# akloetgen/PARA-suite

Hardware: AMD Instinct MI355X
Metric: aligned reads/sec (10Mx50bp PAR-CLIP vs hg19-size genome) on MI355X; SAM bit-exact vs own CPU restatement (parity unpinned) (higher is better)
Workload: dtype u64

## Files before the change

para-suite_amd/csrc/ps_capi.hip:

```cpp
#include <hip/hip_runtime.h>
#include <chrono>
#include <condition_variable>
#include <deque>
#include <functional>
#include <map>
#include <mutex>
#include <thread>
#include <cstdio>
#include <cstdlib>
#include <cstring>
#include <string>
#include <fcntl.h>
#include <unistd.h>
#include "../../include/parasuite_hip.h"
#include "ps_pipeline.h"
#include "ps_bam.h"
#include "ps_host.h"

using namespace ps;

static thread_local std::string g_err;
static int fail(const std::string &m) { g_err = m; std::fprintf(stderr, "[parasuite-hip] error: %s\n", m.c_str()); return 1; }
#define PS_TRY try {
#define PS_CATCH_INT } catch (const std::exception &e) { return fail(e.what()); } catch (...) { return fail("unknown error"); }
// ... 201 lines not shown
int ps_ctx_blob(ps_ctx *x, int which, void **p, uint64_t *bytes)
{
    PS_TRY
        Index &ix = x->c.ix;
        if (which == 0) { *p = ix.blocks.p; *bytes = ix.blocks.n * sizeof(OccBlock); }
        else if (which == 1) { *p = ix.sa.p; *bytes = ix.sa.n * sizeof(uint32_t); }
        else if (which == 2) { *p = ix.pac.p; *bytes = ix.pac.n; }
        else throw Error("blob index out of range");
        return 0;
    PS_CATCH_INT
}
int64_t ps_ctx_meta(ps_ctx *x, char *buf, int64_t cap)
{
    try {
        std::string m = index_meta_serialize(x->c.ix);
        if (buf && cap >= (int64_t)m.size()) std::memcpy(buf, m.data(), m.size());
        return (int64_t)m.size();
    } catch (const std::exception &e) { fail(e.what()); return -1; }
}
ps_ctx *ps_ctx_from_blobs(const char *meta, int64_t meta_len, int device, void *const ptrs[3])
{
    ps_ctx *x = nullptr;
    PS_TRY
        x = new_ctx(device);
        Index &ix = x->c.ix;
        index_meta_deserialize(std::string(meta, (size_t)meta_len), ix);
        const bwtint primary = ix.view.primary; bwtint L2[5]; std::memcpy(L2, ix.view.L2, sizeof L2);
        const size_t nb = ix.view.n_blocks, ns = ix.view.n_sa, np = (size_t)ix.ref.l_pac / 4 + 1;
        ix.blocks.adopt((OccBlock *)ptrs[0], nb); ix.sa.adopt((uint32_t *)ptrs[1], Index::sa_words(ns)); ix.pac.adopt((uint8_t *)ptrs[2], np);
        ix.ref.pac.resize(np);
        PS_HIP(hipMemcpy(ix.ref.pac.data(), ix.pac.p, np, hipMemcpyDeviceToHost));
        ix.refresh_view();
        ix.view.primary = primary; std::memcpy(ix.view.L2, L2, sizeof L2);
        index_build_jump(ix, nullptr);
        return x;
    } catch (const std::exception &e) { delete x; fail(e.what()); return nullptr; } catch (...) { delete x; fail("unknown error"); return nullptr; }
}
int ps_ctx_fetch(ps_ctx *x, int which, void *dst, uint64_t bytes)
{
    PS_TRY
        void *p; uint64_t n;
        if (ps_ctx_blob(x, which, &p, &n)) return 1;
        if (bytes > n) throw Error("fetch larger than blob");
        PS_HIP(hipMemcpy(dst, p, bytes, hipMemcpyDeviceToHost));
        return 0;
    PS_CATCH_INT
}

int ps_ctx_export_blob(ps_ctx *x, int which, void *dst, uint64_t bytes)
{
    PS_TRY
        void *p; uint64_t n;
        if (ps_ctx_blob(x, which, &p, &n)) return 1;
        if (bytes != n) throw Error("export size differs from blob size");
        PS_HIP(hipMemcpy(dst, p, bytes, hipMemcpyDeviceToDevice));
        return 0;
    PS_CATCH_INT
}

ps_batch *ps_batch_from_fastq(ps_ctx *x, const char *fastq)
{
    PS_TRY
        require_device(x->c.device);
        ReadSet rs; load_reads(fastq, rs, x->c.host_threads);
        ps_batch *b = new ps_batch();
        b->b = batch_create(&x->c, std::move(rs));
        return b;
    PS_CATCH_PTR
}
ps_batch *ps_batch_from_codes(ps_ctx *x, int64_t n, int len, const uint8_t *codes)
{
    PS_TRY
        require_device(x->c.device);
        ReadSet rs; reads_from_codes(n, len, codes, rs);
        ps_batch *b = new ps_batch();
        b->b = batch_create(&x->c, std::move(rs));
        return b;
    PS_CATCH_PTR
}
void ps_batch_free(ps_batch *b) { delete b; }
int64_t ps_batch_n(ps_batch *b) { return b->b->rs.n; }
int ps_batch_search(ps_batch *b) { PS_TRY batch_search(*b->b); return 0; PS_CATCH_INT }
int ps_batch_select_hard(ps_batch *b, uint64_t before, uint64_t *after) { PS_TRY batch_select_hard(*b->b, before, after); return 0; PS_CATCH_INT }
int ps_batch_select_easy(ps_batch *b, int threads) { PS_TRY b->b->ctx->host_threads = threads > 0 ? threads : 1; batch_select_easy(*b->b, threads); return 0; PS_CATCH_INT }
int ps_batch_locate(ps_batch *b) { PS_TRY batch_locate(*b->b); return 0; PS_CATCH_INT }
int ps_batch_run(ps_batch *b, int threads)
{
    PS_TRY
        b->b->ctx->host_threads = threads > 0 ? threads : 1;
        batch_search(*b->b);
        batch_select_hard(*b->b, 0, nullptr);
        batch_select_easy(*b->b, threads);
        batch_locate(*b->b);
        return 0;
    PS_CATCH_INT
}
int ps_batch_write_sam(ps_batch *b, const char *path, int with_header, int threads)
{
    PS_TRY
        batch_write_sam(*b->b, path, with_header != 0, "@PG\tID:parasuite-hip\tPN:parasuite-hip\tVN:0.1", threads); return 0;
    PS_CATCH_INT
}
int ps_batch_n_aln(ps_batch *b, int32_t *out, int64_t cap)
{
    PS_TRY
        Batch &B = *b->b;
        for (int64_t g = 0; g < B.rs.n && g < cap; ++g) { int n; B.alns_of(g, n); out[g] = n; }
        return 0;
    PS_CATCH_INT
}
int64_t ps_batch_alns(ps_batch *b, int64_t read, ps_aln *out, int64_t cap)
{
    try {
        int n; const AlnRec *a = b->b->alns_of(read, n);
        for (int j = 0; j < n && j < cap; ++j) std::memcpy(&out[j], &a[j], sizeof(ps_aln));
        return n;
    } catch (const std::exception &e) { fail(e.what()); return -1; }
}
int ps_batch_hits(ps_batch *b, ps_hit *out, int64_t cap)
{
    PS_TRY
        Batch &B = *b->b;
        for (int64_t g = 0; g < B.rs.n && g < cap; ++g) {
            Hit h; B.hit_of(g, h); ps_hit &o = out[g];
            o.pos = h.type ? h.pos : -1; o.sa = h.sa; o.type = h.type; o.strand = h.strand; o.mapq = h.mapq; o.n_mm = h.n_mm; o.n_gapo = h.n_gapo;
            o.n_gape = h.n_gape; o.ref_shift = h.ref_shift; o.score = h.score; o.c1 = h.c1; o.c2 = h.c2; o.n_cigar = h.n_cigar; o.n_multi = h.n_multi;
            std::memset(o.cigar, 0, sizeof o.cigar); std::memcpy(o.cigar, h.cigar, sizeof h.cigar);
        }
        return 0;
    PS_CATCH_INT
}
int64_t ps_ctx_read_iters(ps_ctx *x, uint32_t *out, int64_t cap)
{
    const int64_t n = (int64_t)x->c.read_iters.size();
    for (int64_t i = 0; i < n && i < cap; ++i) out[i] = x->c.read_iters[i];
    return n;
}
int ps_batch_timing(ps_batch *b, ps_timing *o)
{
    PS_TRY
        const Timing &t = b->b->tm;
        o->ms_width = t.ms_width; o->ms_backtrack = t.ms_backtrack; o->ms_compact = t.ms_compact; o->ms_select = t.ms_select;
        o->ms_sa2pos = t.ms_sa2pos; o->ms_refine = t.ms_refine; o->ms_host_post = t.ms_host_post; o->ms_total = t.ms_total;
        o->ms_classify = t.ms_classify; o->ms_rows = t.ms_rows; o->ms_sel_hard = t.ms_sel_hard; o->ms_sel_easy = t.ms_sel_easy;
        o->n_width_launches = t.n_width_launches; o->n_backtrack_launches = t.n_backtrack_launches;
        o->n_overflow_tier1 = b->b->n_overflow[1]; o->n_overflow_tier2 = b->b->n_overflow[2];
        o->bt_begin_ms = t.bt_begin_ms; o->bt_end_ms = t.bt_end_ms;
        return 0;
    PS_CATCH_INT
}
int ps_batch_kstats(ps_batch *b, int which, ps_kstats *o)
{
    PS_TRY
        const KStats &k = which == 0 ? b->b->st_width : (which == 1 ? b->b->st_backtrack : b->b->st_sa2pos);
        o->occ_pairs = k.occ_pairs; o->occ_same_blk = k.occ_same_blk; o->nodes = k.nodes; o->pushes = k.pushes; o->pops = k.pops;
        o->lf_steps = k.lf_steps; o->iters = k.iters; o->exact_steps = k.exact_steps; return 0;
    PS_CATCH_INT
}

static const char *const PS_PG_LINE = "@PG\tID:parasuite-hip\tPN:parasuite-hip\tVN:0.1";
namespace {
struct ProfileSink { int min_mapq = 0, max_len = 0; std::string prefix; };
struct BamOut { int min_mapq = 0; bool sort = false, index = false; int level = 1; BamStats *stats = nullptr;
                bool by_name = false; BamFile *keep = nullptr; };
struct Resident { std::vector<ps_ctx *> xs; bool loaded = false; int n_index_loads = 0; };
struct PassIO { Resident *res = nullptr; std::vector<ReadSet> *reads = nullptr; std::function<void(Batch &)> after_piece; Resident *lanes_from = nullptr;
                int64_t n_reads = 0; double s_parse = 0, s_index = 0; };
}
static int map_core(int threads, const char *mm, const char *error_profile, const char *indel_profile,
                    const char *ref_fa, const char *fastq, const char *out_sam, const ProfileSink *sink, const BamOut *bam = nullptr, PassIO *io = nullptr)
{
    PS_TRY
        const bool verbose = std::getenv("PS_VERBOSE") != nullptr;
        const auto t_begin = std::chrono::steady_clock::now();
        auto since = [&]() { return std::chrono::duration<double>(std::chrono::steady_clock::now() - t_begin).count(); };
        const int nthr = threads > 0 ? threads : 1;
        std::vector<int> devs, dev_workers;
        int per_dev = 1;
        if (const char *e = std::getenv("PS_WORKERS_PER_GPU")) per_dev = std::max(1, std::min(std::atoi(e), (int)Ctx::N_WORK));
        {
            std::vector<int> named;
            if (const char *e = std::getenv("PARASUITE_GPU_IDS")) { for (const char *p = e; *p;) { named.push_back(std::atoi(p)); while (*p && *p != ',') ++p; if (*p == ',') ++p; } }
            else {
                int want = 1, have = 1;
                if (const char *e = std::getenv("PARASUITE_GPUS")) want = std::max(1, std::atoi(e));
                if (want > 1 && (hipGetDeviceCount(&have) != hipSuccess || have < 1)) return fail("no HIP device available");
                for (int g = 0; g < std::min(want, have); ++g) named.push_back(g);
            }
            if (named.empty()) named.push_back(0);
            for (int d : named) {
                size_t k = 0;
                while (k < devs.size() && devs[k] != d) ++k;
                if (k == devs.size()) { devs.push_back(d); dev_workers.push_back(0); }
                ++dev_workers[k];
            }
            for (int &w : dev_workers) w = std::min((int)Ctx::N_WORK, std::max(w, per_dev));
        }
        const int G = (int)devs.size();
        int n_workers = 0; for (int w : dev_workers) n_workers += w;
        size_t chunk_bytes = (size_t)1 << 30, first_bytes = 0, hungry_min = (size_t)128 << 20;
        if (const char *e = std::getenv("PS_CHUNK_MB")) { chunk_bytes = (size_t)std::max(1, std::atoi(e)) << 20; hungry_min = chunk_bytes; }
        else {
            FILE *f = io && io->reads ? nullptr : std::fopen(fastq, "rb");
            if (f) {
                if (fseeko(f, 0, SEEK_END) == 0) {
                    const off_t sz = ftello(f);
                    if (sz > 0) {
                        if (n_workers > 1) chunk_bytes = std::min(chunk_bytes, std::max<size_t>((size_t)16 << 20, ((size_t)sz + 2 * (size_t)n_workers - 1) / (2 * (size_t)n_workers) + ((size_t)64 << 10)));
                        hungry_min = std::min(chunk_bytes, std::max(hungry_min, (size_t)sz / 5));
                        if (bam) { chunk_bytes = std::min(chunk_bytes, std::max<size_t>((size_t)64 << 20, (size_t)sz / 4 + ((size_t)64 << 10))); hungry_min = std::min(hungry_min, chunk_bytes / 2); }
                    }
                }
                std::fclose(f);
            }
        }
        if (const char *e = std::getenv("PS_HUNGRY_MIN_MB")) hungry_min = (size_t)std::max(1, std::atoi(e)) << 20;
        if (const char *e = std::getenv("PS_FIRST_MB")) first_bytes = (size_t)std::max(1, std::atoi(e)) << 20;
        struct Piece { int64_t seq = 0; std::unique_ptr<Batch> b; };
        Chan<Piece> parsed;
        parsed.cap = (size_t)std::max(2, n_workers);
        Resident *const res = io ? io->res : nullptr;
        const bool preloaded = res && res->loaded;
        std::vector<ps_ctx *> xs((size_t)G, nullptr);
        if (res && !res->xs.empty()) { if (res->xs.size() != (size_t)G) return fail("internal: the resident contexts do not match the devices"); xs = res->xs; }
        auto close_all = [&]() { if (res) { res->xs = xs; return; } for (ps_ctx *c : xs) if (c) ps_ctx_close(c); };
        for (int g = 0; g < G; ++g) {
            if (!xs[g]) xs[g] = new_ctx(devs[g], false);
            if (error_profile && error_profile[0] ? ps_ctx_set_profile(xs[g], error_profile, indel_profile, mm)
                                                   : ps_ctx_set_stock(xs[g], mm && mm[0] ? mm : "0.04")) { const std::string m = g_err; close_all(); return fail(m); }
            xs[g]->c.host_threads = nthr;
            xs[g]->c.n_work = dev_workers[g];
        }
        if (res) res->xs = xs;
        if (io && io->lanes_from && io->lanes_from->xs.size() == (size_t)G)
            for (int g = 0; g < G; ++g) {
                Ctx &from = io->lanes_from->xs[g]->c, &to = xs[g]->c;
                if (from.device != to.device) continue;
                std::lock_guard<std::mutex> l1(from.work_mu), l2(to.work_mu);
                for (int w = 0; w < (int)Ctx::N_WORK; ++w) if (from.work[w] && !to.work[w]) to.work[w] = std::move(from.work[w]);
            }
        std::mutex mu; std::condition_variable cv;
        bool failed = false; std::string msg;
        int64_t next_select = 0, write_next = 0; uint64_t draws = 0;
        std::map<int64_t, std::unique_ptr<Batch>> done; int workers_left = n_workers;
        const size_t done_cap = (size_t)n_workers + 2;
        std::vector<int> index_state((size_t)G, preloaded ? 1 : 0);
        std::vector<int> attached((size_t)G, 0);
        auto fail_all = [&](const std::string &m) { { std::lock_guard<std::mutex> l(mu); if (!failed) { failed = true; msg = m; } } cv.notify_all(); parsed.abort(); };
        double t_parse = 0, t_write = 0, t_release = 0, t_index = 0, t_index_all = 0, t_profile = 0; std::vector<double> t_gpu((size_t)n_workers, 0.0);
        int64_t n_reads = 0, n_pieces = 0;
        Trash::trash().collect();
        std::thread parser([&]() {
            try {
                int64_t seq = 0;
                int pthr = nthr;
                if (const char *e = std::getenv("PS_PARSE_THREADS")) pthr = std::max(1, std::atoi(e));
                const std::function<bool()> hungry = [&]() { return parsed.hungry(); };
                if (io && io->reads) {
                    for (ReadSet &rs : *io->reads) { if (rs.n == 0) continue; Piece p; p.seq = seq++; p.b = batch_prepare(&xs[0]->c, std::move(rs), pthr); parsed.push(std::move(p)); }
                    io->reads->clear();
                } else
                load_reads_chunked(fastq, pthr, chunk_bytes, [&](ReadSet &&rs) {
                    Piece p; p.seq = seq++; p.b = batch_prepare(&xs[0]->c, std::move(rs), pthr);
                    parsed.push(std::move(p));
                }, first_bytes, &hungry, hungry_min);
                t_parse = since();
            } catch (const std::exception &e) { fail_all(e.what()); }
            parsed.close();
        });
        std::thread writer([&]() {
            try {
                bool first = true;
                SamScratch scratch;
                if (!bam) { const int fd = ::open(out_sam, O_WRONLY | O_CREAT | O_TRUNC, 0644); if (fd >= 0) ::close(fd); }
                std::unique_ptr<BamSink> bsink;
                std::unique_ptr<ProfileAccum> accum;
                for (;;) {
                    std::unique_ptr<Batch> b;
                    {
                        std::unique_lock<std::mutex> l(mu);
                        cv.wait(l, [&] { return failed || done.count(write_next) || (workers_left == 0 && done.empty()); });
                        if (failed) return;
                        auto it = done.find(write_next);
                        if (it == done.end()) break;
                        b = std::move(it->second); done.erase(it);
                    }
                    const auto t0 = std::chrono::steady_clock::now();
                    if (bam) {
                        if (!bsink) {
                            std::vector<std::pair<std::string, uint32_t>> refs;
                            for (const Contig &ct : b->ctx->ix.ref.contigs) refs.emplace_back(ct.name, (uint32_t)ct.len);
                            bsink.reset(new BamSink(sam_header(b->ctx->ix.ref, PS_PG_LINE), refs, out_sam, bam->sort, bam->index, nthr, bam->level, bam->by_name));
                        }
                        std::vector<std::string> enc; std::vector<std::vector<BamRec>> recs;
                        batch_bam_records(*b, bam->min_mapq, nthr, enc, recs);
                        bsink->add(enc, recs, (uint64_t)b->rs.n);
                    } else batch_write_sam(*b, out_sam, first, PS_PG_LINE, nthr, !first, &scratch);
                    t_write += std::chrono::duration<double>(std::chrono::steady_clock::now() - t0).count();
                    if (sink) {
                        const auto tp = std::chrono::steady_clock::now();
                        if (!accum) accum.reset(new ProfileAccum(xs[0]->c.device, xs[0]->c.ix, sink->max_len));
                        ProfRecords pr;
                        batch_profile_records(*b, sink->min_mapq, nthr, pr);
                        accum->add(pr);
                        t_profile += std::chrono::duration<double>(std::chrono::steady_clock::now() - tp).count();
                    }
                    if (io && io->after_piece) io->after_piece(*b);
// ... 457 lines not shown
```

para-suite_amd/csrc/ps_core.h:

```cpp
#pragma once
#include "ps_types.h"

namespace ps {

PS_HD uint32_t ps_popc(uint32_t x)
{
#ifdef __HIP_DEVICE_COMPILE__
    return (uint32_t)__popc(x);
#else
    return (uint32_t)__builtin_popcount(x);
#endif
}
PS_HD uint32_t pfx_mask32(int ns)
{
    return ns >= 32 ? 0xFFFFFFFFu : (ns <= 0 ? 0u : ((1u << ns) - 1u));
}

struct Blk { uint32_t x[16]; };

#ifdef __HIP_DEVICE_COMPILE__
#define PS_AS_GLOBAL(T, p) ((const __attribute__((address_space(1))) T *)(p))
#define PS_AS_GLOBAL_W(T, p) ((__attribute__((address_space(1))) T *)(p))
typedef uint32_t ps_u32x4 __attribute__((ext_vector_type(4)));
#endif

PS_HD int opaque_lane(int v)
{
#ifdef __HIP_DEVICE_COMPILE__
    asm volatile("" : "+v"(v));
#endif
    return v;
}

PS_HD void load_blk(const OccBlock *blocks, uint32_t b, Blk &o)
{
#ifdef __HIP_DEVICE_COMPILE__
    const __attribute__((address_space(1))) ps_u32x4 *p = PS_AS_GLOBAL(ps_u32x4, blocks + b);
    const ps_u32x4 a = p[0], c = p[1], d = p[2], e = p[3];
    o.x[0] = a.x; o.x[1] = a.y; o.x[2] = a.z; o.x[3] = a.w;
    o.x[4] = c.x; o.x[5] = c.y; o.x[6] = c.z; o.x[7] = c.w;
    o.x[8] = d.x; o.x[9] = d.y; o.x[10] = d.z; o.x[11] = d.w;
    o.x[12] = e.x; o.x[13] = e.y; o.x[14] = e.z; o.x[15] = e.w;
#else
    const uint32_t *p = reinterpret_cast<const uint32_t *>(blocks + b);
    for (int j = 0; j < 16; ++j) o.x[j] = p[j];
#endif
}
PS_HD void blk_count4(const Blk &b, int r, uint32_t cnt[4])
{
    uint32_t c1 = 0, c2 = 0, c3 = 0;
    const int q = r >> 5;
    const uint32_t part = (1u << (r & 31)) - 1u;
#pragma unroll
    for (int j = 0; j < 6; ++j) {
        const uint32_t m = j < q ? 0xFFFFFFFFu : (j == q ? part : 0u), lo = b.x[4 + j] & m, hi = b.x[10 + j] & m;
        c3 += ps_popc(lo & hi);
        c2 += ps_popc(hi & ~lo);
        c1 += ps_popc(lo & ~hi);
    }
    cnt[0] = b.x[0] + ((uint32_t)r - c1 - c2 - c3);
    cnt[1] = b.x[1] + c1; cnt[2] = b.x[2] + c2; cnt[3] = b.x[3] + c3;
}
PS_HD uint32_t blk_count1(const Blk &b, int r, int c)
{
    uint32_t n = 0;
    const uint32_t flo = (c & 1) ? 0u : 0xFFFFFFFFu, fhi = (c & 2) ? 0u : 0xFFFFFFFFu;
#pragma unroll
    for (int j = 0; j < 6; ++j) n += ps_popc((b.x[4 + j] ^ flo) & (b.x[10 + j] ^ fhi) & pfx_mask32(r - 32 * j));
    uint32_t base = c == 0 ? b.x[0] : (c == 1 ? b.x[1] : (c == 2 ? b.x[2] : b.x[3]));
    return base + n;
}
PS_HD int blk_sym(const Blk &b, int pos)
{
    uint32_t lo = 0, hi = 0; const int wi = pos >> 5;
#pragma unroll
    for (int j = 0; j < 6; ++j) { lo = (j == wi) ? b.x[4 + j] : lo; hi = (j == wi) ? b.x[10 + j] : hi; }
    return (int)(((lo >> (pos & 31)) & 1u) | (((hi >> (pos & 31)) & 1u) << 1));
}

PS_HD void blk_pack(OccBlock &b, const uint8_t *syms, int n, const uint32_t cnt[4])
{
    for (int c = 0; c < 4; ++c) b.cnt[c] = cnt[c];
    for (int j = 0; j < 6; ++j) {
        uint32_t lo = 0, hi = 0;
        for (int t = 0; t < 32; ++t) { int p = j * 32 + t; if (p < n) { lo |= (uint32_t)(syms[p] & 1) << t; hi |= (uint32_t)((syms[p] >> 1) & 1) << t; } }
        b.sym[j] = lo; b.sym[6 + j] = hi;
    }
}

PS_HD uint32_t sel4s(uint32_t v0, uint32_t v1, uint32_t v2, uint32_t v3, int c)
{
    const bool b0 = (c & 1) != 0, b1 = (c & 2) != 0;
    const uint32_t lo = b0 ? v1 : v0, hi = b0 ? v3 : v2;
    return b1 ? hi : lo;
}
PS_HD uint32_t sel4(const uint32_t v[4], int c) { return sel4s(v[0], v[1], v[2], v[3], c); }
PS_HD bwtint L2_of(const IndexView &ix, int c)
{
    const bool b0 = (c & 1) != 0, b1 = (c & 2) != 0;
    const bwtint lo = b0 ? ix.L2[1] : ix.L2[0], hi = b0 ? ix.L2[3] : ix.L2[2];
    return b1 ? hi : lo;
}
PS_HD uint32_t cost_word(const uint32_t pk[5], int s)
{
    const uint32_t w = sel4s(pk[0], pk[1], pk[2], pk[3], s);
    return s >= 4 ? pk[4] : w;
}
PS_HD int cost_of(const uint32_t pk[5], int s, int c) { return (int)((cost_word(pk, s) >> (8 * c)) & 0xffu); }

PS_HD bwtint row_to_stored(bwtint primary, bwtint row) { return row - (row >= primary ? 1u : 0u); }
PS_HD uint32_t blk_of(bwtint s, int &off)
{
    const uint32_t b = (uint32_t)(s >> 6) / 3u;
    off = (int)((uint32_t)s - b * (uint32_t)PS_BLK_SYMS);
    return b;
}
PS_HD uint32_t width32(bwtint k, bwtint l) { const bwtint w = l - k + 1; return w > 0xFFFFFFFFull ? 0xFFFFFFFFu : (uint32_t)w; }

struct LaneStats { uint32_t pairs, same, nodes, pushes, pops, iters, exact, lf; };

PS_HD void occ_pair4(const OccBlock *blocks, bwtint primary, bwtint k, bwtint l, uint32_t ck[4], uint32_t cl[4], LaneStats &st)
{
    int ol_ = 0, ok_ = 0;
    const uint32_t bl = blk_of(row_to_stored(primary, l), ol_);
    uint32_t bk = bl;
    bool need_k = k != 0;
    if (need_k) bk = blk_of(row_to_stored(primary, k - 1), ok_);
    Blk xl, xk;
    load_blk(blocks, bl, xl);
    bool other = need_k && bk != bl;
    if (other) load_blk(blocks, bk, xk);
    blk_count4(xl, ol_ + 1, cl);
#pragma unroll
    for (int j = 0; j < 16; ++j) xk.x[j] = other ? xk.x[j] : xl.x[j];
    blk_count4(xk, need_k ? ok_ + 1 : 0, ck);
    if (!need_k) { ck[0] = ck[1] = ck[2] = ck[3] = 0; }
    ++st.pairs;
    if (need_k && !other) ++st.same;
}
PS_HD void occ_pair1(const IndexView &ix, bwtint k, bwtint l, int c, uint32_t &ok, uint32_t &ol, LaneStats &st)
{
    int ol_ = 0, ok_ = 0;
    const uint32_t bl = blk_of(row_to_stored(ix.primary, l), ol_);
    uint32_t bk = bl;
    bool need_k = k != 0;
    if (need_k) bk = blk_of(row_to_stored(ix.primary, k - 1), ok_);
    Blk xl, xk;
    load_blk(ix.blocks, bl, xl);
    bool other = need_k && bk != bl;
    if (other) load_blk(ix.blocks, bk, xk);
    ol = blk_count1(xl, ol_ + 1, c);
    if (!need_k) ok = 0;
    else if (other) ok = blk_count1(xk, ok_ + 1, c);
    else ok = blk_count1(xl, ok_ + 1, c);
    ++st.pairs;
    if (need_k && !other) ++st.same;
}

PS_HD int read_base(const uint32_t *bases, const uint32_t *nmask, int n_reads, int r, int j)
{
    uint32_t w = bases[(size_t)(j >> 4) * n_reads + r];
    uint32_t m = nmask[(size_t)(j >> 5) * n_reads + r];
    return ((m >> (j & 31)) & 1u) ? 4 : (int)((w >> (2 * (j & 15))) & 3u);
}

PS_HD uint8_t cw_pack(int bid, bool eq) { return (uint8_t)((bid > 127 ? 127 : bid) | (eq ? 0x80 : 0)); }

struct WChain { bwtint k, l; int bid; uint32_t prev_w; };
PS_HD void wchain_init(const IndexView &ix, WChain &c) { c.k = 0; c.l = ix.seq_len; c.bid = 0; c.prev_w = 0xFFFFFFFFu; }
PS_HD void wchain_step(const IndexView &ix, WChain &c, int base, uint32_t &w_out, uint8_t &cw_out, bool first, LaneStats &st)
{
    if (base < 4) {
        uint32_t ok, ol;
        occ_pair1(ix, c.k, c.l, base, ok, ol, st);
        const bwtint l2 = L2_of(ix, base);
        c.k = l2 + ok + 1;
        c.l = l2 + ol;
    }
    if (c.k > c.l || base > 3) { c.k = 0; c.l = ix.seq_len; ++c.bid; }
    uint32_t w = width32(c.k, c.l);
    w_out = w;
    cw_out = cw_pack(c.bid, !first && w == c.prev_w);
    c.prev_w = w;
}

static const int PS_POP_TRIES = 1;
enum { M_FETCH = 0, M_POP = 1, M_EXACT = 2, M_EXPAND = 3, M_EXIT = 4, M_HIT = 5,
       M_GROW = 6 };

struct BtLane {
    int r, mode;
    bwtint k, l;
    int i, score, units, n_mm, n_gapo, n_gape, n_ins, n_del, state, ldp;
    bool have_cur;
    int best_score, max_units, n_aln, n_stack, status;
    unsigned long long best_cnt;
    unsigned long long bm0, bm1;
    uint32_t bump, free_head, iters0;
    uint32_t rn0, rn1;
    int len;
    uint32_t n_phantom;
    uint32_t cap;
    LaneStats st;
};

PS_HD int lm_ncw(int len) { return (len + 1 + 3) >> 2; }
PS_HD int lm_ncsw(int seed_len) { return seed_len > 0 ? (seed_len + 1 + 3) >> 2 : 0; }
PS_HD bool lm_nmask_in_regs(int len) { return len <= 64; }
PS_HD int lm_heads_off(int len, int seed_len) { return 4 * (lm_ncw(len) + lm_ncsw(seed_len) + ((len + 15) >> 4) + (lm_nmask_in_regs(len) ? 0 : ((len + 31) >> 5))); }
PS_HD int lm_bytes(int len, int seed_len, int n_buckets, bool wide)
{
    int n = lm_heads_off(len, seed_len) + (wide ? 0 : 2 * n_buckets);
    n = (n + 3) & ~3;
    if (((n >> 2) & 1) == 0) n += 4;
    return n;
}

static const int PS_JUMP_SLOT_WORDS = 8, PS_JUMP_MAX_LEVELS = 14;
PS_HD uint32_t jump_level_off(int d) { return 0x55555555u & ((1u << (2 * d)) - 1u); }
PS_HD size_t jump_words(int levels) { return (size_t)jump_level_off(levels) * PS_JUMP_SLOT_WORDS; }
PS_HD int jump_levels_for(bwtint seq_len) { int k = 0; while (k < PS_JUMP_MAX_LEVELS && (seq_len >> (2 * k)) >= 48) ++k; return k; }

struct BtHot {
    const OccBlock *blocks; bwtint primary;
    const uint32_t *jump; uint32_t jump_levels;
    uint32_t L2lo[4], L2hi;
    uint32_t s_pk[5], u_pk[5];
    uint32_t p0, p1, p2, p3;
    uint32_t inv_c_min, max_entries, pool_cap, n_reads, big_cap;
    uint32_t c_min;
    PS_HD int len() const { return (int)(p0 & 0xffu); }
    PS_HD int seed_len() const { return (int)((p0 >> 8) & 0xffu); }
    PS_HD int indel_end_skip() const { return (int)((p0 >> 16) & 0xffu); }
    PS_HD int max_del_occ() const { return (int)(p0 >> 24); }
    PS_HD int max_gapo() const { return (int)(p1 & 0xfu); }
    PS_HD int max_gape() const { return (int)((p1 >> 4) & 0xfu); }
    PS_HD bool mode_gape() const { return ((p1 >> 8) & 1u) != 0; }
    PS_HD bool use_seed() const { return ((p1 >> 9) & 1u) != 0; }
    PS_HD bool profile() const { return ((p1 >> 10) & 1u) != 0; }
    PS_HD bool has_big() const { return ((p1 >> 11) & 1u) != 0; }
    PS_HD int seed_units() const { return (int)((p1 >> 12) & 0xfffu); }
    PS_HD int u_tight() const { return (int)(p1 >> 24); }
    PS_HD int s_gapo_ins() const { return (int)(p2 & 0xffu); }
    PS_HD int s_gape() const { return (int)((p2 >> 8) & 0xffu); }
    PS_HD int s_gapo_del() const { return (int)((p2 >> 16) & 0xffu); }
    PS_HD int s_stop() const { return (int)(p2 >> 24); }
    PS_HD int u_gapo_ins() const { return (int)(p3 & 0xffu); }
    PS_HD int u_gape() const { return (int)((p3 >> 8) & 0xffu); }
    PS_HD int u_gapo_del() const { return (int)((p3 >> 16) & 0xffu); }
    PS_HD int n_buckets() const { return (int)(p3 >> 24); }
    PS_HD bwtint L2(int c) const
    { return (bwtint)L2lo[c] | ((bwtint)((L2hi >> c) & 1u) << 32); }
    PS_HD bwtint L2_dyn(int c) const
    { return (bwtint)sel4s(L2lo[0], L2lo[1], L2lo[2], L2lo[3], c) | ((bwtint)((L2hi >> c) & 1u) << 32); }
};
inline bool bt_hot_make(const BtArgs &a, BtHot &h)
{
    const Model &md = a.md;
    h.blocks = a.ix.blocks; h.primary = a.ix.primary; h.L2hi = 0;
    h.jump = a.ix.jump; h.jump_levels = a.ix.jump ? (uint32_t)a.ix.jump_levels : 0u;
    for (int c = 0; c < 4; ++c) { h.L2lo[c] = (uint32_t)a.ix.L2[c]; h.L2hi |= (uint32_t)((a.ix.L2[c] >> 32) & 1ull) << c; }
    h.L2hi |= (uint32_t)((a.ix.seq_len >> 32) & 1ull) << 4;
    for (int c = 0; c < 5; ++c) { h.s_pk[c] = md.s_mm_pk[c]; h.u_pk[c] = md.u_mm_pk[c]; }
    const int seed_units = md.max_seed_diff * md.u_tight;
    const bool ok = a.len >= 0 && a.len <= 255 && md.seed_len >= 0 && md.seed_len <= 255 && md.indel_end_skip >= 0 && md.indel_end_skip <= 255 &&
                    md.max_del_occ >= 0 && md.max_del_occ <= 255 && md.max_gapo >= 0 && md.max_gapo <= 15 && md.max_gape >= 0 && md.max_gape <= 15 &&
                    seed_units >= 0 && seed_units <= 4095 && md.u_tight >= 0 && md.u_tight <= 255 && md.s_stop >= 0 && md.s_stop <= 255 &&
                    md.s_gapo_ins >= 0 && md.s_gapo_ins <= 255 && md.s_gape >= 0 && md.s_gape <= 255 && md.s_gapo_del >= 0 && md.s_gapo_del <= 255 &&
                    md.u_gapo_ins >= 0 && md.u_gapo_ins <= 255 && md.u_gape >= 0 && md.u_gape <= 255 && md.u_gapo_del >= 0 && md.u_gapo_del <= 255 &&
                    md.n_buckets >= 0 && md.n_buckets <= 255 && md.max_entries >= 0 && md.inv_c_min >= 0 && md.max_units <= 255 && a.ix.L2[0] == 0;
    h.p0 = (uint32_t)a.len | ((uint32_t)md.seed_len << 8) | ((uint32_t)md.indel_end_skip << 16) | ((uint32_t)md.max_del_occ << 24);
    h.p1 = (uint32_t)md.max_gapo | ((uint32_t)md.max_gape << 4) | ((md.mode_gape ? 1u : 0u) << 8) | ((md.use_seed ? 1u : 0u) << 9) |
// ... 403 lines not shown
```

para-suite_amd/csrc/ps_kernels.h:

```cpp
#pragma once
#include <hip/hip_runtime.h>
#include "ps_types.h"
#include "ps_budget.h"

namespace ps {

static const int PS_MAX_CIGAR = 16;

struct WidthArgs {
    IndexView ix;
    int n_reads, len, seed_len, use_seed;
    const int32_t *lens;
    const uint32_t *bases; const uint32_t *nmask;
    uint32_t *w; uint32_t *cwb; uint32_t *cswb;
    KStats *stats;
};

struct EffortArgs {
    IndexView ix;
    int n_reads, len;
    const int32_t *lens;
    const uint32_t *bases; const uint32_t *nmask;
    uint32_t s_pk[5];
    int c_restart;
    uint32_t w_pin;
    uint8_t *est;
    uint16_t *est_ab;
};

struct EffortModelArgs {
    int n_reads, len;
    const int32_t *lens; const uint8_t *units_by_len;
    const uint32_t *bases; const uint32_t *nmask; const uint32_t *cwb;
    const uint8_t *est;
    uint32_t s_pk[5]; uint32_t inv_c_min;
    int max_units, u_tight, seed_units, use_seed, seed_len;
    int max_gapo, indel_end_skip, u_gapo_ins, u_gapo_del;
    int depth;
    float rows;
    int log_scale;
    uint8_t *key; float *pred;
};

struct RefineItem { int32_t read; bwtint rb; int32_t ref_shift; int32_t strand; };
struct RefineArgs {
    IndexView ix;
    int n_items, len, n_reads;
    const int32_t *lens;
    const uint32_t *bases; const uint32_t *nmask;
    const RefineItem *items;
    uint32_t *cigar; int32_t *n_cigar;
    uint8_t *zbuf; size_t z_per_block;
    int32_t *hebuf; size_t he_per_block;
};
inline size_t refine_he_words(int len) { return (size_t)(len + 2) * 64 * 2; }

static const size_t PS_LDS_PER_CU = 160 * 1024;
void set_dynamic_lds(const void *kernel, const char *name, size_t bytes);

void launch_width(const WidthArgs &a, hipStream_t s);
void launch_effort(const EffortArgs &a, hipStream_t s);
void launch_effort_model(const EffortModelArgs &a, hipStream_t s);
void launch_jump_build(const IndexView &ix, uint32_t *table, int levels, hipStream_t s);
bool launch_backtrack(const BtArgs &a, const BtArgs *d_args , BtArgs *h_stage ,
                      int n_blocks, int lm_stride, hipStream_t s, bool stats);
void launch_index_check(const IndexView &ix, unsigned long long *out , hipStream_t s);
void launch_sa2pos(const IndexView &ix, const bwtint *rows, bwtint *out, int n, KStats *stats, hipStream_t s);
void launch_refine(const RefineArgs &a, int n_blocks, hipStream_t s);
size_t order_sort_tmp_words(int n);
void launch_order_sort(const uint8_t *key, int n, uint32_t *tmp, int32_t *order, hipStream_t s);
void launch_class_ranks(const uint8_t *cls, long long n, const uint32_t *grp, uint32_t *e_before, uint32_t *h_before, hipStream_t s);

}
```

para-suite_amd/csrc/ps_kernels.hip:

```cpp
#include <hip/hip_runtime.h>
#include <algorithm>
#include <cstdlib>
#include <stdexcept>
#include <string>
#include "ps_core.h"
#include "ps_narrow.h"
#include "ps_kernels.h"

namespace ps {

static const int PS_Q_CHUNK = 64;
#ifndef PS_BT_WAVES
#define PS_BT_WAVES 4
#endif

__device__ __forceinline__ unsigned long long wave_sum(unsigned long long v)
{
    for (int o = 32; o > 0; o >>= 1) v += __shfl_xor(v, o, 64);
    return v;
}
__device__ __forceinline__ void flush_stats(KStats *ks, const LaneStats &st)
{
    if (!ks) return;
    unsigned long long v[8] = {st.pairs, st.same, st.nodes, st.pushes, st.pops, st.lf, st.iters, st.exact};
// ... 95 lines not shown
    const unsigned long long t_start = wall_clock64();
    int q_next = 0, q_end = 0;
    bool exhausted = false;
    for (;;) {
        const bool want = L.mode == M_FETCH;
        const unsigned long long wmask = __ballot(want), lmask = __ballot(L.mode != M_EXIT), hmask = __ballot(L.mode == M_HIT);
        if (lmask == 0) break;
        const bool stalled = (wmask | hmask) == lmask;
        const bool serve_hit = hmask != 0 && (__popcll(hmask) >= (int)hit_min || stalled);
        int fetch_r = -1;
        if (wmask) {
            const int cnt = __popcll(wmask);
            if (cnt >= (int)fetch_min || stalled) {
                const int rank = __popcll(wmask & lane_lt);
                int served = 0;
                while (served < cnt) {
                    if (q_next == q_end) {
                        if (exhausted) break;
                        unsigned int base = 0;
                        if (lane == 0) base = atomicAdd(queue, (unsigned int)PS_Q_CHUNK);
                        base = (unsigned int)__shfl((int)base, 0, 64);
                        if (base >= n_reads) { exhausted = true; break; }
                        q_next = (int)base;
                        q_end = (int)base + PS_Q_CHUNK < (int)n_reads ? (int)base + PS_Q_CHUNK : (int)n_reads;
                    }
                    const int take = q_end - q_next < cnt - served ? q_end - q_next : cnt - served;
                    if (want && rank >= served && rank < served + take) fetch_r = q_next + (rank - served);
                    q_next += take; served += take;
                }
                if (want && fetch_r < 0 && exhausted) fetch_r = (int)n_reads;
            }
        }
        bt_iter(a, h, L, m, fetch_r, serve_hit);
    }
    if (lane == 0) L.st.lf = (uint32_t)((wall_clock64() - t_start) >> 4);
    flush_stats(a.stats, L.st);
}


template <bool STATS, bool NB32>
__global__ void __launch_bounds__(256, PS_BT_WAVES) k_backtrack_n(const BtArgs *__restrict__ ap, BtHot hk, int lm_stride)
{
    const BtArgs &a = *ap;
    BtHot h; pin_hot(h, hk);
    uint32_t *const queue = reinterpret_cast<uint32_t *>(pin64(reinterpret_cast<unsigned long long>(a.queue)));
    const uint32_t n_reads = h.n_reads, fetch_min = pin32((uint32_t)a.fetch_min), hit_min = pin32((uint32_t)a.hit_min);
    extern __shared__ __attribute__((aligned(16))) uint8_t smem[];
    const int lane_g = blockIdx.x * blockDim.x + threadIdx.x;
    BtMem m;
    bt_mem_bind(m, smem + (size_t)threadIdx.x * lm_stride, h.len(), h.seed_len());
    uint8_t *const pool_private = reinterpret_cast<uint8_t *>(a.pool) + (size_t)lane_g * h.pool_cap * sizeof(Entry16);
    m.pool = pool_private;
    m.heads = nullptr;
    NLane L;
    nl_init(L);
    LaneStats st;
    ls_init(st);
    NtClock clk;
    for (int j = 0; j < 4; ++j) clk.tm[j] = 0;
    clk.t_last = 0;
#ifdef PS_STAMPS
    clk.t_last = __builtin_amdgcn_s_memtime();
#endif
    const int lane = threadIdx.x & 63;
    const unsigned long long t_start = STATS ? wall_clock64() : 0ull;
    uint32_t iters0 = 0;
    int q_next = 0, q_end = 0;
    bool exhausted = false;
    for (;;) {
        const int mode = nl_mode(L.ctl);
        const bool want = mode == M_FETCH;
        if (want && (L.ctl & NL_BIG)) {
            const unsigned int slot = (unsigned int)((reinterpret_cast<uint8_t *>(m.pool) - a.big_pool) / ((size_t)h.big_cap * sizeof(Entry16)));
            __threadfence();
            atomicExch(a.big_busy + slot, 0u);
            m.pool = pool_private;
            L.ctl &= ~NL_BIG;
        }
        const unsigned long long wmask = __ballot(want), lmask = __ballot(mode != M_EXIT), hmask = __ballot(mode == M_HIT);
        if (lmask == 0) break;
        const bool stalled = (wmask | hmask) == lmask;
        const bool serve_hit = hmask != 0 && (__popcll(hmask) >= (int)hit_min || stalled);
        int fetch_r = -1;
        if (wmask) {
            const int cnt = __popcll(wmask);
            if (cnt >= (int)fetch_min || stalled) {
                const int rank = (int)__builtin_amdgcn_mbcnt_hi((unsigned int)(wmask >> 32), __builtin_amdgcn_mbcnt_lo((unsigned int)wmask, 0u));
                int served = 0;
                while (served < cnt) {
                    if (q_next == q_end) {
                        if (exhausted) break;
                        unsigned int base = 0;
                        if (lane == 0) base = atomicAdd(queue, (unsigned int)PS_Q_CHUNK);
                        base = (unsigned int)__shfl((int)base, 0, 64);
                        if (base >= n_reads) { exhausted = true; break; }
                        q_next = (int)base;
                        q_end = (int)base + PS_Q_CHUNK < (int)n_reads ? (int)base + PS_Q_CHUNK : (int)n_reads;
                    }
                    const int take = q_end - q_next < cnt - served ? q_end - q_next : cnt - served;
                    if (want && rank >= served && rank < served + take) fetch_r = q_next + (rank - served);
                    q_next += take; served += take;
                }
                if (want && fetch_r < 0 && exhausted) fetch_r = (int)n_reads;
            }
        }
        unsigned long long gmask = __ballot(mode == M_GROW);
        while (gmask) {
            const int src = __ffsll((unsigned long long)gmask) - 1;
            gmask &= gmask - 1;
            const unsigned int n_big = a.n_big;
            unsigned int slot = n_big;
            if (lane == src) {
                unsigned int at = atomicAdd(a.big_next, 1u) % n_big;
                for (int tries = 0; tries < 256; ++tries) {
                    if (atomicCAS(a.big_busy + at, 0u, 1u) == 0u) { slot = at; break; }
                    at = at + 1u == n_big ? 0u : at + 1u;
                }
            }
            slot = (unsigned int)__shfl((int)slot, src, 64);
            const unsigned int n_copy = (unsigned int)__shfl((int)nl_bump(L), src, 64);
            const unsigned long long from = (unsigned long long)__shfl((long long)reinterpret_cast<unsigned long long>(m.pool), src, 64);
            if (slot < n_big) {
                const uint4 *sp = reinterpret_cast<const uint4 *>(from);
                uint4 *dp = reinterpret_cast<uint4 *>(a.big_pool + (size_t)slot * h.big_cap * sizeof(Entry16));
                for (unsigned int e = (unsigned int)lane; e < n_copy; e += 64u) dp[e] = sp[e];
                __threadfence();
                if (lane == src) { m.pool = dp; L.ctl = nl_set_mode(L.ctl | NL_BIG, M_EXPAND); }
            } else if (lane == src) L.ctl = nl_set_mode(nl_set_status(L.ctl, RS_OVERFLOW_POOL), M_POP);
        }
        nt_iter<STATS, NB32>(a, h, L, st, m, fetch_r, serve_hit, &clk);
        if (STATS && a.read_iters) {
            const int now = nl_mode(L.ctl);
            if (mode == M_FETCH && now != M_FETCH && now != M_EXIT) {
                iters0 = st.iters - 1u;
                const int len = nl_len(L), sl = h.seed_len();
                a.read_iters[PS_RI_WORDS * (size_t)L.r + 2] = (uint32_t)(m.cw[len - 1] & 0x7f) | ((h.use_seed() && sl > 0 && sl < len ? (uint32_t)(m.csw[sl - 1] & 0x7f) : 0u) << 8) | (a.est_ab ? (uint32_t)a.est_ab[L.r] << 16 : 0u);
                const uint32_t *cw32 = reinterpret_cast<const uint32_t *>(m.cw);
                for (int p = 0; p < 16; ++p) a.read_iters[PS_RI_WORDS * (size_t)L.r + 4 + p] = p < lm_ncw(len) ? cw32[p] : 0u;
            }
            if (mode != M_FETCH && mode != M_EXIT && now == M_FETCH) {
                uint32_t *ri = a.read_iters + PS_RI_WORDS * (size_t)L.r;
                ri[0] = st.iters - iters0; ri[1] = nl_bump(L);
                ri[3] = (uint32_t)nl_best_score(L) | ((uint32_t)nl_max_units(L) << 8) | ((uint32_t)nl_n_aln(L.ctl) << 16);
            }
        }
    }
    if (STATS) {
        if (lane == 0) st.lf = (uint32_t)((wall_clock64() - t_start) >> 4);
#ifdef PS_STAMPS
        st.nodes = lane == 0 ? (uint32_t)(clk.tm[0] >> 6) : 0; st.pushes = lane == 0 ? (uint32_t)(clk.tm[1] >> 6) : 0;
        st.pops = lane == 0 ? (uint32_t)(clk.tm[2] >> 6) : 0; st.exact = lane == 0 ? (uint32_t)(clk.tm[3] >> 6) : 0;
#endif
        flush_stats(a.stats, st);
    } else {
        st.nodes = st.pushes = st.pops = st.iters = st.exact = st.lf = 0;
        flush_stats(a.stats, st);
    }
}

__global__ void __launch_bounds__(256) k_sa2pos(IndexView ix, const bwtint *rows, bwtint *out, int n, KStats *stats)
{
    const int stride = gridDim.x * blockDim.x;
    int item = blockIdx.x * blockDim.x + threadIdx.x;
    LaneStats st = {0, 0, 0, 0, 0, 0, 0, 0};
    bool have = false; bwtint row = 0; uint32_t steps = 0;
    while (true) {
        if (!have) {
            if (item >= n) break;
            row = rows[item]; steps = 0; have = true;
        }
        if (!sa_walk_step(ix, row, steps, st)) {
            out[item] = (bwtint)steps + sa_sample(ix, row / (bwtint)ix.sa_intv);
            item += stride; have = false;
        }
    }
    flush_stats(stats, st);
}

__device__ __forceinline__ int text_sym(const IndexView &ix, bwtint p) { return p < ix.l_pac ? pac_base(ix.pac, p) : 3 - pac_base(ix.pac, 2 * ix.l_pac - 1 - p); }
__global__ void __launch_bounds__(256) k_index_check(IndexView ix, unsigned long long *out)
{
    unsigned long long rows = 0, bad_sym = 0, bad_sa = 0, longest = 0;
    const bwtint n_sa = ix.n_sa;
    for (bwtint t = (bwtint)blockIdx.x * blockDim.x + threadIdx.x; t < n_sa; t += (bwtint)gridDim.x * blockDim.x) {
        bwtint row = t * (bwtint)ix.sa_intv;
        bwtint p = t == 0 ? ix.seq_len : sa_sample(ix, t);
        unsigned long long steps = 0;
        do {
            if (p == 0) {
                if (row != ix.primary) ++bad_sym;
                row = 0; p = ix.seq_len;
            } else {
                if (row == ix.primary) { ++bad_sym; break; }
                int pos = 0;
                const uint32_t b = blk_of(row_to_stored(ix.primary, row), pos);
                Blk x;
                load_blk(ix.blocks, b, x);
                const int c = blk_sym(x, pos);
                if (c != text_sym(ix, p - 1)) ++bad_sym;
                row = L2_of(ix, c) + blk_count1(x, pos + 1, c);
                --p;
            }
            ++steps;
        } while ((row & (bwtint)(ix.sa_intv - 1)) != 0 && steps < 100000ull);
        if ((row & (bwtint)(ix.sa_intv - 1)) != 0) ++bad_sa;
        else {
            const bwtint t2 = row / (bwtint)ix.sa_intv;
            const bwtint want = t2 == 0 ? ix.seq_len : sa_sample(ix, t2);
            if (want != p) ++bad_sa;
        }
        rows += steps;
        if (steps > longest) longest = steps;
    }
    rows = wave_sum(rows); bad_sym = wave_sum(bad_sym); bad_sa = wave_sum(bad_sa);
    for (int o = 32; o > 0; o >>= 1) { const unsigned long long v = __shfl_xor(longest, o, 64); longest = v > longest ? v : longest; }
    if ((threadIdx.x & 63) == 0) { atomicAdd(out + 0, rows); atomicAdd(out + 1, bad_sym); atomicAdd(out + 2, bad_sa); atomicMax(out + 3, longest); }
}
void launch_index_check(const IndexView &ix, unsigned long long *out, hipStream_t s)
{
    hipLaunchKernelGGL(k_index_check, dim3(256 * 16), dim3(256), 0, s, ix, out);
}

__global__ void __launch_bounds__(64) k_refine(RefineArgs a)
{
    int32_t *H = a.hebuf + (size_t)blockIdx.x * a.he_per_block + threadIdx.x;
    int32_t *E = H + (size_t)(a.len + 2) * 64;
    uint8_t *z = a.zbuf + (size_t)blockIdx.x * a.z_per_block + threadIdx.x;
    for (int it = blockIdx.x * 64 + threadIdx.x; it < a.n_items; it += gridDim.x * 64) {
        RefineItem q = a.items[it];
        const int qlen = a.lens ? a.lens[q.read] : a.len;
        int tlen = qlen + q.ref_shift;
        int d = tlen - qlen; if (d < 0) d = -d;
        int w = (int)(d * 1.5); if (w < 50) w = 50;
        const int r = q.read, len = qlen, n_reads = a.n_reads;
        const uint32_t *bases = a.bases, *nmask = a.nmask;
        const int strand = q.strand;
        uint32_t cig[PS_MAX_CIGAR];
        int n = banded_global(len,
            [&](int j) { int b = read_base(bases, nmask, n_reads, r, strand ? len - 1 - j : j); return b > 3 ? 4 : (strand ? 3 - b : b); },
            tlen, a.ix.pac, q.rb, w, H, E, 64, z, 64, cig, PS_MAX_CIGAR);
        a.n_cigar[it] = n;
        for (int j = 0; j < PS_MAX_CIGAR; ++j) a.cigar[(size_t)it * PS_MAX_CIGAR + j] = j < n ? cig[j] : 0;
    }
}

void launch_width(const WidthArgs &a, hipStream_t s)
{
    int blocks = (a.n_reads + 255) / 256;
    if (blocks > 256 * 8) blocks = 256 * 8;
    if (blocks < 1) blocks = 1;
    hipLaunchKernelGGL(k_width, dim3(a.use_seed ? 2 * blocks : blocks), dim3(256), 0, s, a);
}
__global__ void __launch_bounds__(256) k_jump_level(BtHot h, uint32_t *table, bwtint seq_len, int d)
{
    const uint32_t n = 1u << (2 * d);
    for (uint32_t s = blockIdx.x * blockDim.x + threadIdx.x; s < n; s += gridDim.x * blockDim.x) jump_fill_slot(h, table, seq_len, d, s);
}
void launch_jump_build(const IndexView &ix, uint32_t *table, int levels, hipStream_t s)
{
    BtArgs a{};
    a.ix = ix; a.ix.jump = nullptr; a.ix.jump_levels = 0;
    BtHot h;
    (void)bt_hot_make(a, h);
    for (int d = 0; d < levels; ++d) {
        const uint32_t n = 1u << (2 * d);
        const int blocks = (int)std::min<uint32_t>((n + 255u) / 256u, 256u * 16u);
        hipLaunchKernelGGL(k_jump_level, dim3(blocks), dim3(256), 0, s, h, table, ix.seq_len, d);
    }
}
bool launch_backtrack(const BtArgs &a_in, const BtArgs *d_args, BtArgs *h_stage, int n_blocks, int lm_stride, hipStream_t s, bool stats)
{
    BtArgs &a = *h_stage;
    a = a_in;
    const char *ej = std::getenv("PS_JUMP");
    const bool stats_plain = stats && !std::getenv("PS_STATS_JUMP");
    if (stats_plain || a.wide || (ej && std::atoi(ej) == 0)) { a.ix.jump = nullptr; a.ix.jump_levels = 0; }
    BtHot h;
    if (!bt_hot_make(a, h)) return false;
    (void)hipMemcpyAsync(const_cast<BtArgs *>(d_args), &a, sizeof(BtArgs), hipMemcpyHostToDevice, s);
    const size_t lds = (size_t)256 * lm_stride;
    const bool nb32 = a.md.n_buckets <= 32;
    typedef void (*KernelN)(const BtArgs *, BtHot, int);
    const KernelN kn = stats ? (nb32 ? k_backtrack_n<true, true> : k_backtrack_n<true, false>) : (nb32 ? k_backtrack_n<false, true> : k_backtrack_n<false, false>);
    const void *fn = a.wide ? reinterpret_cast<const void *>(k_backtrack_wide) : reinterpret_cast<const void *>(kn);
    set_dynamic_lds(fn, a.wide ? "k_backtrack_wide" : "k_backtrack_n", lds);
    if (a.wide) hipLaunchKernelGGL(k_backtrack_wide, dim3(n_blocks), dim3(256), lds, s, d_args, h, lm_stride);
    else hipLaunchKernelGGL(kn, dim3(n_blocks), dim3(256), lds, s, d_args, h, lm_stride);
    return true;
}
void launch_sa2pos(const IndexView &ix, const bwtint *rows, bwtint *out, int n, KStats *stats, hipStream_t s)
{
    int blocks = (n + 255) / 256;
    if (blocks > 256 * 8) blocks = 256 * 8;
    if (blocks < 1) blocks = 1;
    hipLaunchKernelGGL(k_sa2pos, dim3(blocks), dim3(256), 0, s, ix, rows, out, n, stats);
}
void launch_refine(const RefineArgs &a, int n_blocks, hipStream_t s)
{
    if (!a.hebuf || a.he_per_block < refine_he_words(a.len)) throw std::runtime_error("k_refine: H/E scratch missing or too small");
    hipLaunchKernelGGL(k_refine, dim3(n_blocks), dim3(64), 0, s, a);
}
void set_dynamic_lds(const void *kernel, const char *name, size_t bytes)
{
    if (bytes <= 48 * 1024) return;
    const std::string what = std::string(name) + ": " + std::to_string(bytes) + " B of dynamic LDS";
    if (bytes > PS_LDS_PER_CU) throw std::runtime_error(what + " requested, a CU has " + std::to_string(PS_LDS_PER_CU));
// ... 6 lines not shown
```

para-suite_amd/csrc/ps_narrow.h:

```cpp
#pragma once
#include "ps_core.h"

namespace ps {

PS_HD int nw_i(uint32_t wa) { return (int)(wa & 0xffu); }
PS_HD int nw_ldp(uint32_t wa) { return (int)((wa >> 8) & 0xffu); }
PS_HD int nw_mm(uint32_t wa) { return (int)((wa >> 16) & 0xffu); }
PS_HD int nw_state(uint32_t wa) { return (int)((wa >> 24) & 3u); }
PS_HD int nw_gapo(uint32_t wa) { return (int)((wa >> 26) & 7u); }
PS_HD int nw_gape(uint32_t wa) { return (int)(wa >> 29); }
PS_HD int nw_ins(uint32_t wb) { return (int)(wb & 7u); }
PS_HD int nw_del(uint32_t wb) { return (int)((wb >> 3) & 7u); }
PS_HD uint32_t nw_c(uint32_t wb) { return (wb >> 6) & 7u; }
PS_HD int nw_score(uint32_t wb) { return (int)((wb >> 9) & 0x7fu); }
static const uint32_t NW_KEEP = 0xFCFF0000u;
static const uint32_t NW_C_MASK = 7u << 6;
static const uint32_t NW_ROOT_C = 4u;

PS_HD int nl_mode(uint32_t ctl) { return (int)(ctl & 7u); }
PS_HD uint32_t nl_set_mode(uint32_t ctl, int mode) { return (ctl & ~7u) | (uint32_t)mode; }
static const uint32_t NL_HAVE_CUR = 8u, NL_STATUS = 7u << 4, NL_BIG = 1u << 7;
PS_HD int nl_status(uint32_t ctl) { return (int)((ctl >> 4) & 7u); }
PS_HD uint32_t nl_set_status(uint32_t ctl, int s) { return (ctl & ~NL_STATUS) | ((uint32_t)s << 4); }
PS_HD int nl_n_aln(uint32_t ctl) { return (int)(ctl >> 16); }

struct NLane {
    uint32_t kr, lr, wa, wb;
    uint32_t ctl;
    int r;
    uint32_t lim;
    uint32_t nsb;
    uint32_t n_phantom;
    uint32_t fh;
    uint32_t bm0, bm1;
    uint32_t rn0, rn1;
};
PS_HD int nl_best_score(const NLane &L) { return (int)(L.lim & 0xffu); }
PS_HD int nl_max_units(const NLane &L) { return (int)((L.lim >> 8) & 0xffu); }
PS_HD int nl_len(const NLane &L) { return (int)((L.lim >> 16) & 0xffu); }
PS_HD int nl_n_stack(const NLane &L) { return (int)(L.nsb & 0xffffu); }
PS_HD uint32_t nl_bump(const NLane &L) { return L.nsb >> 16; }
PS_HD uint32_t nl_phantom(const NLane &L) { return L.n_phantom & 0x00FFFFFFu; }
PS_HD int nl_est(const NLane &L) { return (int)(L.n_phantom >> 24); }

PS_HD void nl_init(NLane &L)
{
    L.kr = L.lr = L.wa = L.wb = 0; L.ctl = (uint32_t)M_FETCH; L.r = 0; L.lim = 0; L.nsb = 0;
    L.n_phantom = 0; L.fh = 0xffffu; L.bm0 = L.bm1 = 0; L.rn0 = L.rn1 = 0;
}
PS_HD void ls_init(LaneStats &st) { st.pairs = st.same = st.nodes = st.pushes = st.pops = st.iters = st.exact = st.lf = 0; }
PS_HD uint32_t ps_mul24(uint32_t x, uint32_t y)
{
#ifdef __HIP_DEVICE_COMPILE__
    return __umul24(x, y);
#else
    return x * y;
#endif
}

struct NtClock { unsigned long long tm[4]; unsigned long long t_last; };
#if defined(PS_STAMPS) && defined(__HIP_DEVICE_COMPILE__)
#define PS_USTAMP(clk, slot) do { if (STATS && (clk)) { const unsigned long long t_ = __builtin_amdgcn_s_memtime(); (clk)->tm[slot] += t_ - (clk)->t_last; (clk)->t_last = t_; } } while (0)
#else
#define PS_USTAMP(clk, slot) do { } while (0)
#endif

PS_HD bwtint nt_base(const BtHot &h, uint32_t c)
{
    return (bwtint)sel4s(h.L2lo[0], h.L2lo[1], h.L2lo[2], h.L2lo[3], (int)c) | ((bwtint)((h.L2hi >> c) & 1u) << 32);
}
PS_HD int nt_units(const BtHot &h, uint32_t wa, uint32_t wb)
{
    return h.profile() ? nw_score(wb) : nw_mm(wa) + nw_gapo(wa) + (h.mode_gape() ? nw_gape(wa) : 0);
}

PS_HD void blk_count4b(const Blk &b, int r, uint32_t cnt[4])
{
    uint32_t A = 0, B = 0, C = 0;
    const int q = r >> 5;
    const uint32_t part = (1u << (r & 31)) - 1u;
#pragma unroll
    for (int j = 0; j < 6; ++j) {
        const uint32_t m = j < q ? 0xFFFFFFFFu : (j == q ? part : 0u), lo = b.x[4 + j] & m, hi = b.x[10 + j] & m;
        A += ps_popc(lo); B += ps_popc(hi); C += ps_popc(lo & hi);
    }
    cnt[0] = b.x[0] + ((uint32_t)r - A - B + C);
    cnt[1] = b.x[1] + (A - C); cnt[2] = b.x[2] + (B - C); cnt[3] = b.x[3] + C;
}

#ifndef PS_OCC_COND
#define PS_OCC_COND 1
#endif
template <bool STATS>
PS_HD void nt_occ(const BtHot &h, uint32_t c, uint32_t kr, uint32_t lr, uint32_t ck[4], uint32_t cl[4], LaneStats &st)
{
    const bwtint base = nt_base(h, c);
    const bool need_k = c != NW_ROOT_C;
    int ol_ = 0, ok_ = 0;
    const uint32_t bl = blk_of(row_to_stored(h.primary, base + lr), ol_);
    uint32_t bk = blk_of(row_to_stored(h.primary, base + (bwtint)(need_k ? kr - 1u : 0u)), ok_);
    bk = need_k ? bk : 0u;
    const int rk = need_k ? ok_ + 1 : 0;
    Blk xl, xk;
    load_blk(h.blocks, bl, xl);
    if (PS_OCC_COND) {
        const bool other = bk != bl;
        if (other) load_blk(h.blocks, bk, xk);
        blk_count4b(xl, ol_ + 1, cl);
#pragma unroll
        for (int j = 0; j < 16; ++j) xk.x[j] = other ? xk.x[j] : xl.x[j];
    } else { load_blk(h.blocks, bk, xk); blk_count4b(xl, ol_ + 1, cl); }
    blk_count4b(xk, rk, ck);
    ++st.pairs; if (need_k && bk == bl) ++st.same;
    (void)STATS;
}

PS_HD int nt_depth(int len, uint32_t wa, uint32_t wb) { return len - nw_i(wa) - (int)(wb & 7u) + (int)((wb >> 3) & 7u); }
PS_HD void nt_jump(const BtHot &h, int d, uint32_t sidx, uint32_t ck[4], uint32_t cl[4])
{
    const uint32_t *sl = h.jump + (size_t)(jump_level_off(d) + sidx) * PS_JUMP_SLOT_WORDS;
#ifdef __HIP_DEVICE_COMPILE__
    const ps_u32x4 a = *PS_AS_GLOBAL(ps_u32x4, sl), b = *PS_AS_GLOBAL(ps_u32x4, sl + 4);
    ck[0] = a.x; cl[0] = a.y; ck[1] = a.z; cl[1] = a.w; ck[2] = b.x; cl[2] = b.y; ck[3] = b.z; cl[3] = b.w;
#else
    for (int c = 0; c < 4; ++c) { ck[c] = sl[2 * c]; cl[c] = sl[2 * c + 1]; }
#endif
}
PS_HD void jump_fill_slot(const BtHot &h, uint32_t *table, bwtint seq_len, int d, uint32_t s)
{
    uint32_t c = NW_ROOT_C, kr = 0, lr = (uint32_t)seq_len;
    bool empty = false;
    if (d > 0) {
        const uint32_t *ps = table + (size_t)(jump_level_off(d - 1) + (s >> 2)) * PS_JUMP_SLOT_WORDS;
        c = s & 3u;
        empty = ps[2 * c] >= ps[2 * c + 1];
        kr = ps[2 * c] + 1u; lr = ps[2 * c + 1];
    }
    uint32_t ck[4] = {0, 0, 0, 0}, cl[4] = {0, 0, 0, 0};
    LaneStats st;
    if (!empty) nt_occ<false>(h, c, kr, lr, ck, cl, st);
    uint32_t *out = table + (size_t)(jump_level_off(d) + s) * PS_JUMP_SLOT_WORDS;
    for (int j = 0; j < 4; ++j) { out[2 * j] = ck[j]; out[2 * j + 1] = cl[j]; }
}

PS_HD int nt_seq_at(const BtMem &m, const NLane &L, int j, int len, int max_len)
{
    const int p = len - 1 - j;
    const uint32_t b = (m.rb[p >> 4] >> (2 * (p & 15))) & 3u;
    const uint32_t nw = lm_nmask_in_regs(max_len) ? (p < 32 ? L.rn0 : L.rn1) : m.rn[p >> 5];
    return ((nw >> (p & 31)) & 1u) ? 4 : 3 - (int)b;
}

PS_HD void nt_heads_init(BtMem &m, int n_buckets)
{
    uint32_t *hw = reinterpret_cast<uint32_t *>(m.heads16);
    for (int p = 0; p < (n_buckets + 1) >> 1; ++p) hw[p] = 0xFFFFFFFFu;
}
PS_COLD void nt_restart_without_estimate(const BtArgs &a, NLane &L, BtMem &m)
{
    L.ctl = (L.ctl & NL_BIG) | (uint32_t)M_POP | NL_HAVE_CUR;
    L.kr = 0; L.lr = (uint32_t)a.ix.seq_len; L.wa = (uint32_t)nl_len(L); L.wb = NW_ROOT_C << 6;
    L.lim = (L.lim & 0x00FFFF00u) | 0xffu;
    L.nsb = 0; L.bm0 = L.bm1 = 0; L.fh = 0xffffu; L.n_phantom = 0xFF000000u;
    nt_heads_init(m, a.md.n_buckets);
}
PS_HD void nt_finish_read(const BtArgs &a, NLane &L)
{
    a.n_aln[L.r] = nl_n_aln(L.ctl);
    a.status[L.r] = (uint8_t)nl_status(L.ctl);
    L.ctl = nl_set_mode(L.ctl, M_FETCH);
}

PS_COLD void nt_hit(const BtArgs &a, NLane &L, BtMem &m)
{
    const Model &md = a.md;
    const uint32_t c = nw_c(L.wb);
    if (a.ix.jump && c != NW_ROOT_C) {
        const int d = nt_depth(nl_len(L), L.wa, L.wb);
        if (d < a.ix.jump_levels) {
            const uint32_t *ps = a.ix.jump + (size_t)(jump_level_off(d - 1) + (L.kr >> 2)) * PS_JUMP_SLOT_WORDS;
            L.kr = ps[2 * c] + 1u; L.lr = ps[2 * c + 1];
        }
    }
    const bwtint base = c == NW_ROOT_C ? (a.ix.seq_len & ~(bwtint)0xFFFFFFFFull) : a.ix.L2[c];
    const bwtint k = base + L.kr, l = base + L.lr;
    const int score = nw_score(L.wb), n_gapo = nw_gapo(L.wa);
    const int units = md.profile ? score : nw_mm(L.wa) + n_gapo + (md.mode_gape ? nw_gape(L.wa) : 0);
    const int n_aln = nl_n_aln(L.ctl);
    if (n_aln == 0) {
        if (units > nl_est(L)) { nt_restart_without_estimate(a, L, m); return; }
        int t = units + md.u_tight;
        const int own = nl_max_units(L);
        t = t > own ? own : t;
        L.lim = (L.lim & 0x00FF0000u) | (uint32_t)score | ((uint32_t)t << 8);
    }
    if (score == nl_best_score(L)) {
        const unsigned long long s = (unsigned long long)(L.lim >> 24) + (unsigned long long)(l - k) + 1ull;
        L.lim = (L.lim & 0x00FFFFFFu) | ((s > 255ull ? 255u : (uint32_t)s) << 24);
    } else if ((int)(L.lim >> 24) > md.max_top2) { nt_finish_read(a, L); return; }
    AlnRec *out = a.alns + (size_t)L.r * a.aln_cap;
    if (n_gapo) {
        for (int j = 0; j < n_aln; ++j)
            if (out[j].k == k && out[j].l == l) return;
    }
    {
        const uint32_t shadow = a.ix.seq_len > 0xFFFFFFFFull ? 0xFFFFFFFFu : (uint32_t)a.ix.seq_len;
        uint32_t x = (uint32_t)(l - k + 1), j = 0, prev = 0;
        const int lim = nw_ldp(L.wa);
        for (int i = 0; i < lim; ++i) {
            size_t off = (size_t)i * a.n_reads + L.r;
            uint32_t w = a.w[off];
            int bid = m.cw[i] & 0x7f;
            if (w > x) { w -= x; a.w[off] = w; }
            else if (w == x) {
                if (bid > 1 && nl_phantom(L)) L.ctl = nl_set_status(L.ctl, RS_OVERFLOW_POOL);
                bid = 1; w = shadow - (++j); a.w[off] = w;
            }
            m.cw[i] = cw_pack(bid, i > 0 && w == prev);
            prev = w;
        }
        if (lim > 0) {
            uint32_t w = a.w[(size_t)lim * a.n_reads + L.r];
            m.cw[lim] = cw_pack(m.cw[lim] & 0x7f, w == prev);
        }
    }
    if (n_aln >= a.aln_cap) { L.ctl = nl_set_status(L.ctl, RS_OVERFLOW_ALN); nt_finish_read(a, L); return; }
    AlnRec rec;
    rec.k = k; rec.l = l; rec.score = (uint16_t)score; rec.units = (uint16_t)units;
    rec.n_mm = (uint8_t)nw_mm(L.wa); rec.n_gapo = (uint8_t)n_gapo; rec.n_gape = (uint8_t)nw_gape(L.wa);
    rec.n_ins = (uint8_t)nw_ins(L.wb); rec.n_del = (uint8_t)nw_del(L.wb);
    for (int j = 0; j < 7; ++j) rec.pad[j] = 0;
    out[n_aln] = rec;
    L.ctl += 1u << 16;
}

PS_COLD bool nt_fetch(const BtArgs &a, NLane &L, BtMem &m, int q)
{
    const Model &md = a.md;
    const int r = a.order ? a.order[q] : q;
    const int len = a.lens ? a.lens[r] : a.len;
    L.r = r;
    L.ctl = (uint32_t)M_FETCH;
    L.n_phantom = 0xFF000000u;
    const int max_units = (a.lens && a.units_by_len) ? (int)a.units_by_len[len] : md.max_units;
    L.lim = 0xffu | ((uint32_t)max_units << 8) | ((uint32_t)len << 16);
    {
        const int ncw = lm_ncw(len), ncsw = lm_ncsw(md.seed_len);
        uint32_t *cw32 = reinterpret_cast<uint32_t *>(m.cw), *csw32 = reinterpret_cast<uint32_t *>(m.csw);
        for (int p = 0; p < ncw; ++p) cw32[p] = a.cwb[(size_t)p * a.n_reads + r];
        for (int p = 0; p < ncsw; ++p) csw32[p] = a.cswb[(size_t)p * a.n_reads + r];
        const int nbw = (len + 15) >> 4;
        for (int p = 0; p < nbw; ++p) m.rb[p] = a.bases[(size_t)p * a.n_reads + r];
    }
    int nNu = 0;
    L.rn0 = L.rn1 = 0;
    const int nmw = (len + 31) >> 5;
    for (int p = 0; p < nmw; ++p) {
        uint32_t w = a.nmask[(size_t)p * a.n_reads + r];
        if (lm_nmask_in_regs(a.len)) { if (p == 0) L.rn0 = w; else L.rn1 = w; }
        else m.rn[p] = w;
        nNu += (int)ps_popc(w) * (int)(md.u_mm_pk[4] & 0xffu);
    }
    if (nNu > max_units) { nt_finish_read(a, L); return false; }
    L.kr = 0; L.lr = (uint32_t)a.ix.seq_len; L.wa = (uint32_t)len; L.wb = NW_ROOT_C << 6;
    L.ctl |= NL_HAVE_CUR;
    L.nsb = 0; L.bm0 = L.bm1 = 0; L.fh = 0xffffu;
    {
        int e = 255;
        if (a.cap_est) { e = (int)a.est[r] - (a.cap_est - 1); if (e < 0) e = 0; }
        L.n_phantom = (uint32_t)(e + md.u_tight < max_units ? e : 255) << 24;
    }
    nt_heads_init(m, md.n_buckets);
    return true;
}

PS_HD uint32_t nt_slot(NLane &L)
{
    const uint32_t fr = L.fh;
    const bool reuse = fr != 0xffffu;
    const uint32_t idx = reuse ? fr : (L.nsb >> 16);
    L.nsb += reuse ? 1u : 0x10001u;
    L.fh = 0xffffu;
    return idx;
}
PS_HD void nt_push(NLane &L, BtMem &m, uint32_t kr, uint32_t lr, uint32_t wa, uint32_t wb)
{
    const int score = nw_score(wb);
    const uint32_t idx = nt_slot(L);
    const uint32_t next = (uint32_t)m.heads16[score];
    Entry16 e; e.k = kr; e.l = lr; e.a = wa; e.b = wb | (next << 16);
    store16(reinterpret_cast<Entry16 *>(m.pool) + idx, e);
    m.heads16[score] = (uint16_t)idx;
    if (score < 32) L.bm0 |= 1u << score; else L.bm1 |= 1u << (score - 32);
}

template <bool NB32>
PS_HD void nt_pop(NLane &L, BtMem &m)
{
#ifdef __HIP_DEVICE_COMPILE__
    const int b = (NB32 || L.bm0) ? __ffs((int)L.bm0) - 1 : 32 + __ffs((int)L.bm1) - 1;
#else
    const int b = (NB32 || L.bm0) ? __builtin_ctz(L.bm0) : 32 + __builtin_ctz(L.bm1);
#endif
    const uint32_t hd = m.heads16[b];
    Entry16 e;
    load16(reinterpret_cast<const Entry16 *>(m.pool) + hd, e);
    const uint32_t next = e.b >> 16;
    L.fh = hd;
    m.heads16[b] = (uint16_t)next;
    if (next == PS_NIL16) { if (NB32 || b < 32) L.bm0 &= ~(1u << b); else L.bm1 &= ~(1u << (b - 32)); }
    L.kr = e.k; L.lr = e.l; L.wa = e.a; L.wb = e.b & 0xffffu;
    L.nsb -= 1u;
}

template <bool STATS, bool NB32>
PS_HD int nt_head(const BtArgs &a, const BtHot &h, NLane &L, LaneStats &st, BtMem &m, int fetch_r, bool serve_hit)
{
    int mode = nl_mode(L.ctl);
    if (mode == M_EXIT || mode == M_GROW) return 0;
    if (STATS) ++st.iters;
    if (mode == M_HIT) {
        if (!serve_hit) return 0;
        L.ctl = nl_set_mode(L.ctl, M_POP);
        { NLane t = L; nt_hit(a, t, m); L = t; }
        return 0;
    }
    if (mode == M_FETCH) {
        if (fetch_r < 0) return 0;
        if (fetch_r >= (int)h.n_reads) { L.ctl = nl_set_mode(L.ctl, M_EXIT); return 0; }
        { NLane t = L; const bool ok = nt_fetch(a, t, m, fetch_r); L = t; if (!ok) return 0; }
        L.ctl = nl_set_mode(L.ctl, M_POP);
        mode = M_POP;
    }
    if (mode == M_POP) {
        const int n_virtual = nl_n_stack(L) + ((L.ctl & NL_HAVE_CUR) ? 1 : 0);
        if (nl_phantom(L) && (long long)n_virtual + (long long)nl_phantom(L) > (long long)h.max_entries) {
            L.ctl = nl_set_status(L.ctl, RS_OVERFLOW_POOL); nt_finish_read(a, L); return 0;
        }
        if (n_virtual == 0 && nl_est(L) != 255 && nl_n_aln(L.ctl) == 0 && nl_status(L.ctl) == RS_OK) { NLane t = L; nt_restart_without_estimate(a, t, m); L = t; return 0; }
        if (n_virtual == 0 || n_virtual > (int)h.max_entries || nl_status(L.ctl) != RS_OK) { nt_finish_read(a, L); return 0; }
        if (L.ctl & NL_HAVE_CUR) L.ctl &= ~NL_HAVE_CUR;
        else { nt_pop<NB32>(L, m); if (STATS) ++st.pops; }
        L.ctl = nl_set_mode(L.ctl, M_POP);
        const int score = nw_score(L.wb), i1 = nw_i(L.wa);
        if (score > nl_best_score(L) + h.s_stop()) { nt_finish_read(a, L); return 0; }
        const int rem = nl_max_units(L) - nt_units(h, L.wa, L.wb);
        if (rem < 0) return 0;
        const int mleft = (int)(ps_mul24((uint32_t)rem, h.inv_c_min) >> 16);
        if (i1 > 0 && mleft < (int)(m.cw[i1 - 1] & 0x7f)) return 0;
        if (i1 == 0) { L.ctl = nl_set_mode(L.ctl, M_HIT); return 0; }
        const int st_ = nw_state(L.wa);
        mode = (mleft == 0 && (st_ == ST_M || h.mode_gape() || nw_gape(L.wa) == h.max_gape())) ? M_EXACT : M_EXPAND;
    }
    return mode;
}

struct NtStep { uint32_t ck[4], cl[4]; uint32_t cw_i, cw_im1, cs_i, cs_im1; int s, i; bool in_seed, tm, ctm; };

template <bool STATS>
PS_HD void nt_step_occ(const BtHot &h, NLane &L, LaneStats &st, BtMem &m, NtStep &q)
{
    const int len = nl_len(L), max_len = h.len();
    const int i = nw_i(L.wa) - 1;
    q.i = i;
    q.cw_i = m.cw[i]; q.cw_im1 = m.cw[i > 0 ? i - 1 : 0];
    const int ii = i - (len - h.seed_len());
    q.in_seed = h.use_seed() && len > h.seed_len() && ii > 0;
    q.cs_i = q.in_seed ? m.csw[ii] : 0u; q.cs_im1 = q.in_seed ? m.csw[ii - 1] : 0u;
    q.s = nt_seq_at(m, L, i, len, max_len);
    const int depth = nt_depth(len, L.wa, L.wb);
    q.tm = depth < (int)h.jump_levels; q.ctm = depth + 1 < (int)h.jump_levels;
    if (!q.tm) nt_occ<STATS>(h, nw_c(L.wb), L.kr, L.lr, q.ck, q.cl, st);
    else nt_jump(h, depth, L.kr, q.ck, q.cl);
}

template <bool STATS, bool NB32>
PS_HD void nt_tail(const BtHot &h, NLane &L, LaneStats &st, BtMem &m, const NtStep &q, int mode)
{
    const int len = nl_len(L), i = q.i, s = q.s;
    const uint32_t cw_i = q.cw_i, cw_im1 = q.cw_im1, cs_i = q.cs_i, cs_im1 = q.cs_im1;
    const bool in_seed = q.in_seed, tm = q.tm, ctm = q.ctm;
    uint32_t ck[4], cl[4];
#pragma unroll
    for (int c = 0; c < 4; ++c) { ck[c] = q.ck[c]; cl[c] = q.cl[c]; }
    if (mode == M_EXACT) {
        if (STATS) ++st.exact;
        L.ctl = nl_set_mode(L.ctl, M_POP);
        if (s > 3) return;
        const uint32_t ok = sel4(ck, s), ol = sel4(cl, s);
        if (ok >= ol) return;
        L.kr = ctm ? (L.kr << 2) | (uint32_t)s : ok + 1u; L.lr = ctm ? ol - ok : ol; L.wa -= 1u; L.wb = (L.wb & ~NW_C_MASK) | ((uint32_t)s << 6);
        L.ctl = nl_set_mode(L.ctl, i == 0 ? M_HIT : M_EXACT);
        return;
    }
    if (STATS) ++st.nodes;
    const uint32_t cap = (L.ctl & NL_BIG) ? h.big_cap : h.pool_cap;
    if (nl_bump(L) + 9u > cap) {
        if (!(L.ctl & NL_BIG) && h.has_big()) { L.ctl = nl_set_mode(L.ctl, M_GROW); return; }
        L.ctl = nl_set_mode(nl_set_status(L.ctl, cap >= 65535u ? RS_OVERFLOW_DEEP : RS_OVERFLOW_POOL), M_POP); return;
    }
    const int max_units = nl_max_units(L);
    const int e_un = nt_units(h, L.wa, L.wb), e_sc = nw_score(L.wb);
    const int rem = max_units - e_un;
    const uint32_t inv = h.inv_c_min;
    const int mleft = (int)(ps_mul24((uint32_t)rem, inv) >> 16);
    const int srem = h.seed_units() - e_un;
    const int m_seed = srem <= 0 ? 0 : (int)(ps_mul24((uint32_t)srem, inv) >> 16);
    bool allow_diff = true, allow_M = true;
    const int bnd_same = i > 0 ? (int)(cw_im1 & 0x7f) : 0;
    const int bnd_del = (int)(cw_i & 0x7f);
    if (i > 0) {
        if (bnd_same > mleft - 1) allow_diff = false;
        else if (bnd_same == mleft - 1 && bnd_del == mleft - 1 && (cw_i & 0x80u)) allow_M = false;
        if (in_seed) {
            const int s1 = (int)(cs_im1 & 0x7f), s0 = (int)(cs_i & 0x7f);
            if (s1 > m_seed - 1) allow_diff = false;
            else if (s1 == m_seed - 1 && s0 == m_seed - 1 && (cs_i & 0x80u)) allow_M = false;
        }
    }
    const int e_go = nw_gapo(L.wa), e_ge = nw_gape(L.wa), e_st = nw_state(L.wa);
    const int tmp = e_go + e_ge;
    const bool gap_ok = allow_diff && i >= h.indel_end_skip() + tmp && len - i >= h.indel_end_skip() + tmp;
    const bool from_m = e_st == ST_M, from_i = e_st == ST_I, from_d = e_st == ST_D;
    const uint32_t wa_keep = L.wa & NW_KEEP, pos2 = (uint32_t)i | ((uint32_t)i << 8);
    const uint32_t wb0 = L.wb & 0x1ffu;
    const uint32_t pkr = L.kr, plr = L.lr;
    const int need_same = (int)ps_mul24((uint32_t)bnd_same, h.c_min), need_del = (int)ps_mul24((uint32_t)bnd_del, h.c_min);
    const int cap_rem = nl_est(L) - e_sc, ut = h.u_tight();
    const int cap_same = cap_rem + (ut > need_same ? ut - need_same : 0), cap_del = cap_rem + (ut > need_del ? ut - need_del : 0);
    const int thr_same = (rem - need_same) < cap_same ? (rem - need_same) : cap_same, thr_del = (rem - need_del) < cap_del ? (rem - need_del) : cap_del;
    uint32_t phantom = 0, gmask = 0;
    int sc[9];
    uint32_t wa_i, wa_d;
    {
        const bool open = from_m && e_go < h.max_gapo(), ext = from_i && e_ge < h.max_gape();
        const int c = open ? h.u_gapo_ins() : h.u_gape();
        sc[0] = e_sc + (open ? h.s_gapo_ins() : h.s_gape());
        const bool cand = gap_ok && (open || ext) && c <= rem, go = cand && c <= thr_same;
        gmask |= go ? 1u : 0u;
        phantom += (cand && !go) ? 1u : 0u;
        wa_i = wa_keep + pos2 + ((uint32_t)ST_I << 24) + (open ? 1u << 26 : 1u << 29);
    }
    {
        const uint32_t occ = tm ? plr : plr - pkr + 1u;
        const bool open = from_m && e_go < h.max_gapo();
        const bool ext = from_d && e_ge < h.max_gape() && ((e_ge + e_go) * h.u_tight() < max_units || occ < (uint32_t)h.max_del_occ());
        const int c = open ? h.u_gapo_del() : h.u_gape();
        const int scd = e_sc + (open ? h.s_gapo_del() : h.s_gape());
        const bool cand = gap_ok && (open || ext) && c <= rem, go = cand && c <= thr_del;
        const uint32_t ne = (ck[0] < cl[0] ? 2u : 0u) | (ck[1] < cl[1] ? 4u : 0u) | (ck[2] < cl[2] ? 8u : 0u) | (ck[3] < cl[3] ? 16u : 0u);
        gmask |= go ? ne : 0u;
        if (cand && !go) phantom += ps_popc(ne);
        sc[1] = sc[2] = sc[3] = sc[4] = scd;
        wa_d = wa_keep + ((uint32_t)(i + 1) | ((uint32_t)(i + 1) << 8)) + ((uint32_t)ST_D << 24) + (open ? 1u << 26 : 1u << 29);
    }
    const bool do_mm = allow_diff && allow_M;
    const uint32_t s_word = cost_word(h.s_pk, s), u_word = h.profile() ? s_word : cost_word(h.u_pk, s);
    uint32_t xk[4], xl[4];
#pragma unroll
    for (int j = 1; j <= 4; ++j) {
        const int c = (s + j) & 3;
        xk[j - 1] = sel4(ck, c); xl[j - 1] = sel4(cl, c);
        sc[4 + j] = 0;
        if (j < 4 || s > 3) {
            const int cu = (int)((u_word >> (8 * c)) & 0xffu);
            sc[4 + j] = e_sc + (int)((s_word >> (8 * c)) & 0xffu);
            const bool cand = do_mm && xk[j - 1] < xl[j - 1] && cu <= rem, go = cand && cu <= thr_same;
            gmask |= go ? 1u << (4 + j) : 0u;
            phantom += (cand && !go) ? 1u : 0u;
        }
    }
    const uint32_t n_push = ps_popc(gmask), fr = L.fh;
    const bool reuse = fr != 0xffffu && n_push != 0u;
    const uint32_t slot0 = (L.nsb >> 16) - (reuse ? 1u : 0u);
    L.nsb += n_push + ((n_push - (reuse ? 1u : 0u)) << 16);
    L.fh = n_push ? 0xffffu : fr;
    if (STATS) st.pushes += n_push;
    uint32_t idx[9], raw[9];
#pragma unroll
    for (int j = 0; j < 9; ++j) {
        idx[j] = 0; raw[j] = 0;
        if ((gmask >> j) & 1u) {
            const uint32_t rank = ps_popc(gmask & ((1u << j) - 1u));
            idx[j] = (reuse && rank == 0u) ? fr : slot0 + rank;
            raw[j] = m.heads16[sc[j]];
            m.heads16[sc[j]] = (uint16_t)idx[j];
            if (NB32 || sc[j] < 32) L.bm0 |= 1u << sc[j]; else L.bm1 |= 1u << (sc[j] - 32);
        }
    }
#ifdef __HIP_DEVICE_COMPILE__
    asm volatile("" : "+v"(raw[0]), "+v"(raw[1]), "+v"(raw[2]), "+v"(raw[3]), "+v"(raw[4]), "+v"(raw[5]), "+v"(raw[6]), "+v"(raw[7]), "+v"(raw[8]));
#endif
    Entry16 *const pool = reinterpret_cast<Entry16 *>(m.pool);
#define NT_NEXT(j) (raw[j] << 16)
    if (gmask & 1u) { Entry16 e; e.k = pkr; e.l = plr; e.a = wa_i; e.b = (wb0 + 1u) | ((uint32_t)sc[0] << 9) | NT_NEXT(0); store16(pool + idx[0], e); }
    {
        const uint32_t wb_d = ((wb0 & 0x3fu) + (1u << 3)) | ((uint32_t)sc[1] << 9);
#pragma unroll
        for (int c = 0; c < 4; ++c)
            if ((gmask >> (1 + c)) & 1u) { Entry16 e; e.k = ctm ? (pkr << 2) | (uint32_t)c : ck[c] + 1u; e.l = ctm ? cl[c] - ck[c] : cl[c]; e.a = wa_d; e.b = wb_d | ((uint32_t)c << 6) | NT_NEXT(1 + c); store16(pool + idx[1 + c], e); }
    }
    {
// ... 34 lines not shown
```

para-suite_amd/csrc/ps_pipeline.h:

```cpp
#pragma once
#include <functional>
#include <map>
#include <memory>
#include <mutex>
#include "ps_host.h"
#include "ps_reads.h"
#include "ps_bam.h"

namespace ps {

static const int PS_HIT_CIGAR = 8;
struct Multi { int64_t pos; bwtint row; int32_t gap, mm, ref_shift, strand, n_cigar; uint32_t cigar[PS_MAX_CIGAR]; };
struct Hit {
    int64_t pos; bwtint sa;
    int32_t type, strand, mapq, n_mm, n_gapo, n_gape, ref_shift, score, c1, c2, n_cigar;
    int32_t multi_begin, n_multi;
    uint32_t cigar[PS_HIT_CIGAR];
};

static const uint8_t PS_CLS_HOST = 4;
struct SelRec { bwtint sa; int32_t c1, c2; uint8_t type, n_mm, n_gapo, n_gape; int8_t ref_shift; uint8_t score, pad[2]; };
struct FinRec { int64_t pos; uint8_t strand, mapq, type, pad[5]; };
struct DevCigar { int64_t g; int32_t n; uint32_t c[PS_HIT_CIGAR]; };
struct SubRead { int64_t g = 0, easy_before = 0, hard_before = 0; uint8_t cls = 0; const AlnRec *alns = nullptr; int32_t n_alns = 0; Hit hit; };

struct Timing {
    double ms_width = 0, ms_backtrack = 0, ms_compact = 0, ms_select = 0, ms_sa2pos = 0, ms_refine = 0, ms_host_post = 0, ms_total = 0, ms_classify = 0, ms_rows = 0, ms_sel_hard = 0, ms_sel_easy = 0;
    int n_width_launches = 0, n_backtrack_launches = 0;
    double bt_begin_ms = 0, bt_end_ms = 0;
};

void *pin_cache_take(size_t need, size_t &got);
void pin_cache_give(void *p, size_t bytes);
void pin_cache_release();
struct PinBuf {
    void *p = nullptr; size_t bytes = 0;
    PinBuf() {}
    PinBuf(const PinBuf &) = delete;
    PinBuf &operator=(const PinBuf &) = delete;
    ~PinBuf() { if (p) pin_cache_give(p, bytes); }
    void *get(size_t need) { if (need > bytes) { if (p) pin_cache_give(p, bytes); p = nullptr; bytes = 0; p = pin_cache_take(need, bytes); } return p; }
};

struct Work {
    hipStream_t stream = nullptr;
    std::map<std::string, DevBuf<uint8_t>> ws; std::map<std::string, PinBuf> pin;
    template <class T> T *ws_get(const std::string &name, size_t count) {
        DevBuf<uint8_t> &b = ws[name];
        const size_t need = count * sizeof(T);
        if (b.n < need) b.alloc(need + need / 8);
        return reinterpret_cast<T *>(b.p);
    }
    template <class T> T *pin_get(const std::string &name, size_t count) { return reinterpret_cast<T *>(pin[name].get(count * sizeof(T) + 64)); }
    Work() {}
    Work(const Work &) = delete;
    Work &operator=(const Work &) = delete;
    ~Work() { if (stream) (void)hipStreamDestroy(stream); }
};

struct Ctx {
    int device = 0;
    hipStream_t stream = nullptr;
    hipEvent_t ref_event = nullptr;
    Index ix;
    Options opt;
    int bt_blocks = 0;
    uint32_t pool_cap[3] = {16384, 65535, 2000064};
    int aln_cap[3] = {8, 256, 65536};
    int aln_cap_short = 32;
    bool want_kstats = false;
    bool want_read_iters = false; std::vector<uint32_t> read_iters;
    int n_big = 4096;
    int fetch_min = 8, hit_min = 1;
    int host_threads = 8;
    static const int N_WORK = 4;
    std::unique_ptr<Work> work[N_WORK];
    int n_work = 1, next_work = 0;
    Work *take_work();
    Work *work_at(int i);
    std::mutex work_mu;
    ~Ctx();
};

struct Bin {
    int len = 0; Model md;
    bool ragged = false;
    std::vector<int32_t> lens; DevBuf<int32_t> d_lens;
    std::vector<int32_t> ids;
    DevBuf<uint32_t> bases, nmask, w; DevBuf<uint8_t> cwb, cswb, status; DevBuf<AlnRec> alns; DevBuf<int32_t> n_aln;
    RawVec<uint32_t> h_bases, h_nmask;
    DevBuf<int32_t> d_ids;
    DevBuf<AlnRec> d_alns; DevBuf<int32_t> d_n_aln; DevBuf<uint8_t> d_status; int aln_cap = 0;
    bool host_alns_valid = false;
    std::vector<int32_t> h_n_aln; std::vector<uint32_t> h_off; std::vector<AlnRec> h_alns;
    std::map<int32_t, std::vector<AlnRec>> overflow;
    int n_bw = 0, n_mw = 0;
};

struct Batch {
    Ctx *ctx = nullptr;
    Work *wk = nullptr;
    int work_index = -1;
    ReadSet rs;
    std::vector<Bin> bins;
    std::vector<int32_t> read_bin, read_local;
    DevBuf<uint8_t> d_class; DevBuf<uint32_t> d_eb, d_hb; DevBuf<bwtint> d_rows, d_pos; DevBuf<SelRec> d_sel; DevBuf<FinRec> d_fin;
    PinBuf p_class, p_sel, p_fin, p_grp;
    uint8_t *h_class = nullptr; SelRec *h_sel = nullptr; FinRec *h_fin = nullptr;
    uint32_t *h_grp = nullptr;
    std::vector<SubRead> sub; std::vector<Multi> multis; std::vector<DevCigar> dev_cigars;
    std::vector<std::unique_ptr<PinBuf>> sub_alns;
    int64_t n_class1 = 0, n_hard = 0;
    std::vector<uint64_t> hard_draws_cum;
    uint64_t draws_in = 0, draws_out = 0;
    DevBuf<KStats> d_stats; KStats st_width{}, st_backtrack{}, st_sa2pos{};
    Timing tm;
    int64_t n_overflow[3] = {0, 0, 0};
    bool searched = false, selected_hard = false, selected = false, located = false;
    const AlnRec *alns_of(int64_t g, int &n);
    void ensure_host_alns();
    void hit_of(int64_t g, Hit &h) const;
    void release_device();
};

std::unique_ptr<Batch> batch_create(Ctx *ctx, ReadSet &&rs);
std::unique_ptr<Batch> batch_prepare(Ctx *ctx, ReadSet &&rs, int threads);
void batch_upload(Batch &b);
void batch_search(Batch &b);
void batch_select_hard(Batch &b, uint64_t draws_before, uint64_t *draws_after);
void batch_select_easy(Batch &b, int threads);
void ctx_release_device(Ctx &c);
void reserve_search_workspace(Ctx *ctx, int work_index);
void batch_locate(Batch &b);
void batch_bam_records(const Batch &b, int min_mapq, int threads, std::vector<std::string> &enc, std::vector<std::vector<BamRec>> &recs);
std::string sam_header(const RefSeq &ref, const char *pg_line);
struct SamScratch { std::vector<std::string> bufs[2]; };
void batch_write_sam(Batch &b, const char *path, bool header, const char *pg_line, int threads, bool append = false, SamScratch *scratch = nullptr);
void batch_profile_records(const Batch &b, int min_mapq, int threads, ProfRecords &out);

}
```

para-suite_amd/csrc/ps_pipeline.hip:

```cpp
#include <hip/hip_runtime.h>
#include <mutex>
#include <optional>
#include <hipcub/hipcub.hpp>
#include <algorithm>
#include <atomic>
#include <chrono>
#include <cmath>
#include <cstdio>
#include <cstring>
#include <functional>
#include <thread>
#include "ps_pipeline.h"
#include "ps_par.h"
#include "ps_core.h"

namespace ps {

typedef std::chrono::steady_clock Clock;
static double ms_since(Clock::time_point t0) { return std::chrono::duration<double, std::milli>(Clock::now() - t0).count(); }

void require_device(int device)
{
    int n = 0;
    hipError_t e = hipGetDeviceCount(&n);
// ... 46 lines not shown
            return p;
        }
    }
    const size_t want = need + need / 8 + 4096;
    void *p = nullptr;
    PS_HIP(hipHostMalloc(&p, want, hipHostMallocDefault));
    got = want;
    return p;
}
void pin_cache_give(void *p, size_t bytes)
{
    if (!p) return;
    PinCache &c = pin_cache();
    {
        std::lock_guard<std::mutex> l(c.mu);
        if (c.held + bytes <= PinCache::CAP) { c.kept.emplace_back(p, bytes); c.held += bytes; return; }
    }
    (void)hipHostFree(p);
}
void pin_cache_release()
{
    PinCache &c = pin_cache();
    std::vector<std::pair<void *, size_t>> all;
    { std::lock_guard<std::mutex> l(c.mu); all.swap(c.kept); c.held = 0; }
    for (auto &e : all) (void)hipHostFree(e.first);
}

void Batch::release_device()
{
    for (Bin &bin : bins) {
        bin.bases.release(); bin.nmask.release(); bin.w.release(); bin.cwb.release(); bin.cswb.release(); bin.status.release();
        bin.alns.release(); bin.n_aln.release(); bin.d_lens.release(); bin.d_ids.release();
        bin.d_alns.release(); bin.d_n_aln.release(); bin.d_status.release();
    }
    d_class.release(); d_eb.release(); d_hb.release(); d_rows.release(); d_pos.release(); d_sel.release(); d_fin.release(); d_stats.release();
    searched = false;
}

std::unique_ptr<Batch> batch_prepare(Ctx *ctx, ReadSet &&rs_in, int threads)
{
    const auto t_prep0 = std::chrono::steady_clock::now();
    struct PrepTimes { double bins = 0, sort = 0, pack = 0; } pt;
    std::unique_ptr<Batch> b(new Batch());
    b->ctx = ctx; b->rs = std::move(rs_in);
    const ReadSet &rs = b->rs;
    std::vector<int> class_of_len;
    std::map<std::vector<int>, int> bin_of_class;
    b->read_bin.resize((size_t)rs.n); b->read_local.resize((size_t)rs.n);
    for (int64_t g = 0; g < rs.n; ++g) {
        const int len = rs.len[g];
        if (len < 1) throw Error("empty read in input");
        if ((size_t)len >= class_of_len.size()) class_of_len.resize((size_t)len + 64, -1);
        int cls = class_of_len[(size_t)len];
        if (cls < 0) {
            Model md; std::string err;
            if (!make_model(ctx->opt, len, md, err)) throw Error(err);
            const std::vector<int> key = {md.max_gapo};
            auto bc = bin_of_class.find(key);
            if (bc == bin_of_class.end()) { bc = bin_of_class.emplace(key, (int)b->bins.size()).first; b->bins.emplace_back(); }
            cls = class_of_len[(size_t)len] = bc->second;
        }
        Bin &bin = b->bins[(size_t)cls];
        if (bin.len && bin.len != len) bin.ragged = true;
        if (len > bin.len) bin.len = len;
        b->read_bin[g] = cls; b->read_local[g] = (int32_t)bin.ids.size();
        bin.ids.push_back((int32_t)g);
    }
    pt.bins = std::chrono::duration<double>(std::chrono::steady_clock::now() - t_prep0).count();
    for (Bin &bin : b->bins) {
        std::string err;
        if (!make_model(ctx->opt, bin.len, bin.md, err)) throw Error(err);
        if (!std::getenv("PS_KEEP_ORDER")) {
            const size_t n = bin.ids.size();
            const int nt = par_threads(n, threads);
            std::vector<uint32_t> key(n), key2(n); std::vector<int32_t> id2(n);
            par_for(n, nt, [&](size_t r0, size_t r1, int) {
                for (size_t r = r0; r < r1; ++r) {
                    const uint8_t *sq = rs.seq.data() + rs.off[bin.ids[r]];
                    const int kb = rs.len[bin.ids[r]] < 16 ? rs.len[bin.ids[r]] : 16;
                    uint32_t k = 0;
                    for (int j = 0; j < kb; ++j) k = (k << 2) | (uint32_t)(sq[j] & 3);
                    key[r] = k << (2 * (16 - kb));
                }
            });
            std::vector<size_t> cnt((size_t)nt * 256);
            for (int sh = 0; sh < 32; sh += 8) {
                std::fill(cnt.begin(), cnt.end(), 0);
                par_for(n, nt, [&](size_t r0, size_t r1, int t) { size_t *c = cnt.data() + (size_t)t * 256; for (size_t r = r0; r < r1; ++r) ++c[(key[r] >> sh) & 0xff]; });
                size_t at = 0;
                for (int d = 0; d < 256; ++d) for (int t = 0; t < nt; ++t) { const size_t c = cnt[(size_t)t * 256 + d]; cnt[(size_t)t * 256 + d] = at; at += c; }
                par_for(n, nt, [&](size_t r0, size_t r1, int t) {
                    size_t *c = cnt.data() + (size_t)t * 256;
                    for (size_t r = r0; r < r1; ++r) { const size_t p = c[(key[r] >> sh) & 0xff]++; key2[p] = key[r]; id2[p] = bin.ids[r]; }
                });
                key.swap(key2); bin.ids.swap(id2);
            }
            par_for(n, nt, [&](size_t r0, size_t r1, int) { for (size_t r = r0; r < r1; ++r) b->read_local[bin.ids[r]] = (int32_t)r; });
        }
        const size_t n = bin.ids.size();
        pt.sort = std::chrono::duration<double>(std::chrono::steady_clock::now() - t_prep0).count() - pt.bins - pt.pack;
        bin.n_bw = (bin.len + 15) / 16; bin.n_mw = (bin.len + 31) / 32;
        bin.h_bases.resize((size_t)bin.n_bw * n); bin.h_nmask.resize((size_t)bin.n_mw * n);
        bin.lens.resize(n);
        {
            const int nt = std::max(1, std::min(threads, 64));
            auto pack = [&](int t) {
                const size_t r_end = n * (t + 1) / nt, AHEAD = 12;
                for (size_t r = n * t / nt; r < r_end; ++r) {
                    if (r + 2 * AHEAD < r_end) { const int32_t g2 = bin.ids[r + 2 * AHEAD]; __builtin_prefetch(&rs.off[g2]); __builtin_prefetch(&rs.len[g2]); }
                    if (r + AHEAD < r_end) { const uint8_t *q = rs.seq.data() + rs.off[bin.ids[r + AHEAD]]; __builtin_prefetch(q); __builtin_prefetch(q + 63); }
                    const uint8_t *s = rs.seq.data() + rs.off[bin.ids[r]];
                    const int rl = rs.len[bin.ids[r]];
                    bin.lens[r] = rl;
                    for (int p = 0; p < bin.n_bw; ++p) {
                        uint32_t wd = 0;
                        const int j1 = std::min(rl, 16 * p + 16);
                        for (int j = 16 * p; j < j1; ++j) if (s[j] <= 3) wd |= (uint32_t)s[j] << (2 * (j & 15));
                        bin.h_bases[(size_t)p * n + r] = wd;
                    }
                    for (int p = 0; p < bin.n_mw; ++p) {
                        uint32_t wd = 0;
                        const int j1 = std::min(rl, 32 * p + 32);
                        for (int j = 32 * p; j < j1; ++j) if (s[j] > 3) wd |= 1u << (j & 31);
                        bin.h_nmask[(size_t)p * n + r] = wd;
                    }
                }
            };
            std::vector<std::thread> th;
            for (int t = 1; t < nt; ++t) th.emplace_back(pack, t);
            pack(0);
            for (auto &x : th) x.join();
        }
        pt.pack = std::chrono::duration<double>(std::chrono::steady_clock::now() - t_prep0).count() - pt.bins - pt.sort;
    }
    if (const char *e = std::getenv("PS_VERBOSE")) if (std::atoi(e) >= 2)
        std::fprintf(stderr, "[parasuite-hip]     piece of %lld reads made ready in %.0f ms (bins %.0f, leading-base sort %.0f, packing %.0f)\n", (long long)rs.n,
                     1e3 * std::chrono::duration<double>(std::chrono::steady_clock::now() - t_prep0).count(), 1e3 * pt.bins, 1e3 * pt.sort, 1e3 * pt.pack);
    return b;
}
void batch_upload(Batch &bb)
{
    Batch *b = &bb; Ctx *ctx = b->ctx;
    require_device(ctx->device);
    b->wk = b->work_index >= 0 ? ctx->work_at(b->work_index) : ctx->take_work();
    Work *wk = b->wk;
    for (Bin &bin : b->bins) {
        const size_t n = bin.ids.size();
        if (bin.ragged) { bin.d_lens.alloc(n); bin.d_lens.upload(bin.lens.data(), n, wk->stream); }
        bin.d_ids.alloc(n); bin.d_ids.upload(bin.ids.data(), n, wk->stream);
        bin.bases.alloc(bin.h_bases.size()); bin.nmask.alloc(bin.h_nmask.size());
        bin.bases.upload(bin.h_bases.data(), bin.h_bases.size(), wk->stream);
        bin.nmask.upload(bin.h_nmask.data(), bin.h_nmask.size(), wk->stream);
    }
    b->d_stats.alloc(3);
    PS_HIP(hipStreamSynchronize(wk->stream));
}
std::unique_ptr<Batch> batch_create(Ctx *ctx, ReadSet &&rs_in)
{
    std::unique_ptr<Batch> b = batch_prepare(ctx, std::move(rs_in), ctx->host_threads);
    batch_upload(*b);
    return b;
}

__global__ void k_gather_alns(const AlnRec *alns, int aln_cap, const int32_t *n_aln, const uint32_t *off, int n, AlnRec *out)
{
    for (int r = blockIdx.x * blockDim.x + threadIdx.x; r < n; r += gridDim.x * blockDim.x) {
        int m = n_aln[r]; if (m > aln_cap) m = aln_cap;
        for (int j = 0; j < m; ++j) out[off[r] + j] = alns[(size_t)r * aln_cap + j];
    }
}
__global__ void k_clip_counts(const int32_t *n_aln, int aln_cap, int n, uint32_t *out)
{
    for (int r = blockIdx.x * blockDim.x + threadIdx.x; r < n; r += gridDim.x * blockDim.x) { int m = n_aln[r]; out[r] = (uint32_t)(m > aln_cap ? aln_cap : (m < 0 ? 0 : m)); }
}

__global__ void k_order_keys(const uint8_t *est, int n, int cap, uint8_t *key)
{
    for (int r = blockIdx.x * blockDim.x + threadIdx.x; r < n; r += gridDim.x * blockDim.x) {
        const int e = est[r] > cap ? cap : est[r];
        key[r] = (uint8_t)(cap - e);
    }
}

struct EvTimer {
    hipEvent_t a, b; hipStream_t s;
    explicit EvTimer(hipStream_t st) : s(st) { PS_HIP(hipEventCreate(&a)); PS_HIP(hipEventCreate(&b)); PS_HIP(hipEventRecord(a, s)); }
    double stop() { mark(); return read(); }
    void mark() { PS_HIP(hipEventRecord(b, s)); }
    double read() { PS_HIP(hipEventSynchronize(b)); float ms = 0; PS_HIP(hipEventElapsedTime(&ms, a, b)); return ms; }
    void span(hipEvent_t ref, double &t_begin, double &t_end) { float x = 0, y = 0; if (ref && hipEventElapsedTime(&x, ref, a) == hipSuccess && hipEventElapsedTime(&y, ref, b) == hipSuccess) { t_begin = x; t_end = y; } }
    ~EvTimer() { (void)hipEventDestroy(a); (void)hipEventDestroy(b); }
};


static void run_search(Batch &b, const Model &md, int n, const uint32_t *d_bases, const uint32_t *d_nmask, const int32_t *d_lens,
                       uint32_t pool_cap, int aln_cap, AlnRec *alns, int32_t *n_aln, uint8_t *status, bool first_tier = false)
{
    Ctx *ctx = b.ctx; Work *wk = b.wk; hipStream_t s = wk->stream;
    const int len = md.len, seed_len = md.seed_len;
    uint32_t *w = wk->ws_get<uint32_t>("w", (size_t)(len + 1) * n);
    uint32_t *cwb = wk->ws_get<uint32_t>("cwb", (size_t)lm_ncw(len) * n);
    uint32_t *cswb = wk->ws_get<uint32_t>("cswb", (size_t)(lm_ncsw(seed_len) + 1) * n);
    WidthArgs wa;
    wa.ix = ctx->ix.view; wa.n_reads = n; wa.len = len; wa.lens = d_lens; wa.seed_len = seed_len; wa.use_seed = md.use_seed;
    wa.bases = d_bases; wa.nmask = d_nmask; wa.w = w; wa.cwb = cwb; wa.cswb = cswb; wa.stats = b.d_stats.p + 0;
    std::optional<EvTimer> t_width, t_order;
    t_width.emplace(s); launch_width(wa, s); PS_HIP(hipGetLastError()); t_width->mark(); ++b.tm.n_width_launches;
    const bool wide = launch_is_wide(md, pool_cap);
    const int32_t *d_order = nullptr; const uint8_t *d_est = nullptr; const uint16_t *d_est_ab = nullptr;
    if (!wide) {
        const char *eo = std::getenv("PS_ORDER");
        const int mode = eo ? std::atoi(eo) : 1;
        int min_n = 4096;
        if (const char *e = std::getenv("PS_ORDER_MIN")) min_n = std::max(1, std::atoi(e));
        if (mode > 0 && n >= min_n && md.max_units >= md.c_min) {
            t_order.emplace(s);
            uint8_t *est = wk->ws_get<uint8_t>("est", (size_t)n), *key = wk->ws_get<uint8_t>("okey", (size_t)n);
            int32_t *order = wk->ws_get<int32_t>("order", (size_t)n);
            EffortArgs ea;
            ea.ix = ctx->ix.view; ea.n_reads = n; ea.len = len; ea.lens = d_lens; ea.bases = d_bases; ea.nmask = d_nmask; ea.est = est;
            int csum = 0;
            for (int c = 0; c < 5; ++c) ea.s_pk[c] = md.u_mm_pk[c];
            for (int sc = 0; sc < 4; ++sc) for (int tc = 0; tc < 4; ++tc) if (sc != tc) csum += md.u_mm[sc][tc];
            ea.c_restart = std::max(1, (csum + 6) / 12);
            if (const char *e = std::getenv("PS_ORDER_RESTART")) ea.c_restart = std::max(1, std::atoi(e));
            ea.w_pin = 16;
            if (const char *e = std::getenv("PS_ORDER_WPIN")) ea.w_pin = (uint32_t)std::max(1, std::atoi(e));
            int lv = 0; while (lv < 31 && (ctx->ix.view.seq_len >> (2 * lv)) > 0) ++lv;
            ea.est_ab = ctx->want_read_iters ? wk->ws_get<uint16_t>("est_ab", (size_t)n) : nullptr;
            launch_effort(ea, s);
            d_est_ab = ea.est_ab;
            if (mode == 2) {
                int cap = 255;
                if (const char *e = std::getenv("PS_ORDER_CAP")) cap = std::max(1, std::min(255, std::atoi(e)));
                hipLaunchKernelGGL(k_order_keys, dim3(std::min((n + 255) / 256, 4096)), dim3(256), 0, s, est, n, cap, key);
            } else {
                EffortModelArgs em;
                em.n_reads = n; em.len = len; em.lens = d_lens; em.units_by_len = nullptr; em.bases = d_bases; em.nmask = d_nmask; em.cwb = cwb; em.est = est;
                for (int c = 0; c < 5; ++c) em.s_pk[c] = md.u_mm_pk[c];
                em.inv_c_min = (uint32_t)md.inv_c_min; em.max_units = md.max_units; em.u_tight = md.u_tight;
                em.seed_units = md.max_seed_diff * md.u_tight; em.use_seed = md.use_seed; em.seed_len = md.seed_len;
                em.max_gapo = md.max_gapo; em.indel_end_skip = md.indel_end_skip; em.u_gapo_ins = md.u_gapo_ins; em.u_gapo_del = md.u_gapo_del;
                em.depth = lv + 3; em.rows = (float)ctx->ix.view.seq_len; em.log_scale = 8;
                if (const char *e = std::getenv("PS_ORDER_SCALE")) em.log_scale = std::max(1, std::min(12, std::atoi(e)));
                if (d_lens) {
                    uint8_t *tab = wk->pin_get<uint8_t>("units_by_len_h2", 256);
                    for (int l2 = 0; l2 < 256; ++l2) { const int u = budget_diffs(ctx->opt, l2) * (ctx->opt.profile ? ctx->opt.unit : 1); tab[l2] = (uint8_t)(u > 255 ? 255 : u); }
                    uint8_t *d_tab = wk->ws_get<uint8_t>("units_by_len2", 256);
                    PS_HIP(hipMemcpyAsync(d_tab, tab, 256, hipMemcpyHostToDevice, s));
                    em.units_by_len = d_tab;
                }
                em.key = key; em.pred = nullptr;
                launch_effort_model(em, s);
            }
            launch_order_sort(key, n, wk->ws_get<uint32_t>("order_tmp", order_sort_tmp_words(n)), order, s);
            PS_HIP(hipGetLastError());
            t_order->mark();
            d_order = order; d_est = est;
        }
    }
    int dev_cus = 256;
    { hipDeviceProp_t p; if (hipGetDeviceProperties(&p, ctx->device) == hipSuccess && p.multiProcessorCount > 0) dev_cus = p.multiProcessorCount; }
    const int lm = lm_bytes(len, seed_len, md.n_buckets, wide);
    int per_cu = (int)((size_t)(160 * 1024) / ((size_t)256 * lm));
    if (per_cu < 1) throw Error("read length / score range too large for the per-lane LDS state");
    { const char *e = std::getenv("PS_MAX_PER_CU"); const int cap = e ? std::atoi(e) : 4; if (per_cu > cap) per_cu = cap; }
    int blocks = ctx->bt_blocks > 0 ? ctx->bt_blocks : dev_cus * per_cu;
    int need = (n + 255) / 256;
    if (blocks > need) blocks = need;
    const size_t per_lane = (size_t)pool_cap * (wide ? sizeof(Entry) : 16) + (wide ? PS_MAX_BUCKETS * 4 : 0);
    const size_t max_lanes = ((size_t)(wide ? 32 : 64) << 30) / per_lane;
    if ((size_t)blocks * 256 > max_lanes) blocks = (int)std::max<size_t>(1, max_lanes / 256);
    const int n_lanes = blocks * 256;
    uint8_t *pool = wk->ws_get<uint8_t>("pool", (size_t)n_lanes * pool_cap * (wide ? sizeof(Entry) : 16));
    uint32_t *heads = wide ? wk->ws_get<uint32_t>("heads", (size_t)n_lanes * PS_MAX_BUCKETS) : nullptr;
    uint32_t *queue = wk->ws_get<uint32_t>("queue", 16);
    PS_HIP(hipMemsetAsync(queue, 0, 64, s));
    BtArgs a; std::memset(&a, 0, sizeof a);
    a.ix = ctx->ix.view; a.md = md; a.n_reads = n; a.len = len; a.lens = d_lens; a.n_lanes = n_lanes;
    if (d_lens) {
        uint8_t *tab = wk->pin_get<uint8_t>("units_by_len_h", 256);
        for (int l2 = 0; l2 < 256; ++l2) { const int u = budget_diffs(ctx->opt, l2) * (ctx->opt.profile ? ctx->opt.unit : 1); tab[l2] = (uint8_t)(u > 255 ? 255 : u); }
        uint8_t *d_tab = wk->ws_get<uint8_t>("units_by_len", 256);
        PS_HIP(hipMemcpyAsync(d_tab, tab, 256, hipMemcpyHostToDevice, s));
        a.units_by_len = d_tab;
    }
    a.bases = d_bases; a.nmask = d_nmask; a.n_bw = (len + 15) / 16; a.n_mw = (len + 31) / 32;
    a.w = w; a.cwb = cwb; a.cswb = cswb;
    a.alns = alns; a.aln_cap = aln_cap; a.n_aln = n_aln; a.status = status;
    a.pool = pool; a.pool_cap = pool_cap; a.heads = heads; a.wide = wide ? 1 : 0; a.stats = b.d_stats.p + 1;
    a.queue = queue; a.fetch_min = ctx->fetch_min; a.hit_min = ctx->hit_min;
    a.order = d_order; a.est = d_est; a.est_ab = d_est_ab;
    a.cap_est = (first_tier && !wide && d_est && md.profile && !(std::getenv("PS_CAP") && std::atoi(std::getenv("PS_CAP")) == 0)) ? 1 : 0;
    if (a.cap_est) if (const char *e = std::getenv("PS_CAP_BIAS")) a.cap_est += std::max(0, std::min(200, std::atoi(e)));
    if (const char *e = std::getenv("PS_FETCH_MIN")) a.fetch_min = std::max(1, std::atoi(e));
    if (const char *e = std::getenv("PS_HIT_MIN")) a.hit_min = std::max(1, std::atoi(e));
    if (!wide && pool_cap < 65535 && ctx->n_big > 0) {
        a.big_cap = 65535; a.n_big = (uint32_t)std::min<int64_t>(ctx->n_big, std::max(64, n));
        a.big_pool = wk->ws_get<uint8_t>("big_pool", (size_t)a.n_big * a.big_cap * 16);
        a.big_next = queue + 4;
        a.big_busy = wk->ws_get<uint32_t>("big_busy", a.n_big);
        PS_HIP(hipMemsetAsync(a.big_busy, 0, (size_t)a.n_big * 4, s));
    }
    uint32_t *riters = nullptr;
    if (ctx->want_read_iters) { riters = wk->ws_get<uint32_t>("riters", (size_t)n * PS_RI_WORDS); PS_HIP(hipMemsetAsync(riters, 0, (size_t)n * PS_RI_WORDS * 4, s)); a.read_iters = riters; }
    { EvTimer t(s);
      if (!launch_backtrack(a, wk->ws_get<BtArgs>("btargs", 1), wk->pin_get<BtArgs>("btargs_h", 1), blocks, lm, s, ctx->want_kstats || ctx->want_read_iters)) throw Error("cost model outside the ranges the search kernel packs (gap/score fields must fit a byte)");
      PS_HIP(hipGetLastError());
      const double ms = t.stop(); b.tm.ms_backtrack += ms; ++b.tm.n_backtrack_launches;
      b.tm.ms_width += t_width->read();
      if (t_order) b.tm.ms_width += t_order->read();
      { double t0_ = 0, t1_ = 0; t.span(ctx->ref_event, t0_, t1_); if (b.tm.n_backtrack_launches == 1) b.tm.bt_begin_ms = t0_; b.tm.bt_end_ms = t1_; }
      if (std::getenv("PS_VERBOSE")) std::fprintf(stderr, "[parasuite-hip]   backtrack launch: %d reads x %d bp, stack %u%s, %d lanes, %.1f ms\n", n, len, pool_cap, wide ? " (wide)" : "", n_lanes, ms); }
    if (ctx->want_read_iters) { ctx->read_iters.resize((size_t)n * PS_RI_WORDS); PS_HIP(hipMemcpyAsync(ctx->read_iters.data(), riters, (size_t)n * PS_RI_WORDS * 4, hipMemcpyDeviceToHost, s)); PS_HIP(hipStreamSynchronize(s)); }
}

static void download_alns(Work *wk, int n, int aln_cap, const AlnRec *d_alns, const int32_t *d_n_aln,
                          std::vector<int32_t> &n_aln, std::vector<uint32_t> &off, std::vector<AlnRec> &alns)
{
    hipStream_t s = wk->stream;
    uint32_t *cnt = wk->ws_get<uint32_t>("cnt", n), *d_off = wk->ws_get<uint32_t>("off", (size_t)n + 1);
    hipLaunchKernelGGL(k_clip_counts, dim3((n + 255) / 256), dim3(256), 0, s, d_n_aln, aln_cap, n, cnt);
    size_t tb = 0;
    PS_HIP(hipcub::DeviceScan::ExclusiveSum(nullptr, tb, cnt, d_off, n, s));
    uint8_t *tmp = wk->ws_get<uint8_t>("scan_tmp", tb ? tb : 1);
    PS_HIP(hipcub::DeviceScan::ExclusiveSum(tmp, tb, cnt, d_off, n, s));
    int32_t *p_na = wk->pin_get<int32_t>("dl_n_aln", n); uint32_t *p_off = wk->pin_get<uint32_t>("dl_off", (size_t)n + 1);
    PS_HIP(hipMemcpyAsync(p_na, d_n_aln, (size_t)n * 4, hipMemcpyDeviceToHost, s));
    PS_HIP(hipMemcpyAsync(p_off, d_off, (size_t)n * 4, hipMemcpyDeviceToHost, s));
    PS_HIP(hipStreamSynchronize(s));
    uint32_t last = 0;
    if (n) { int m = p_na[n - 1]; last = p_off[n - 1] + (uint32_t)(m > aln_cap ? aln_cap : (m < 0 ? 0 : m)); }
    p_off[n] = last;
    n_aln.assign(p_na, p_na + n); off.assign(p_off, p_off + n + 1); alns.resize(last);
    if (last) {
        AlnRec *comp = wk->ws_get<AlnRec>("comp", last);
        hipLaunchKernelGGL(k_gather_alns, dim3((n + 255) / 256), dim3(256), 0, s, d_alns, aln_cap, d_n_aln, d_off, n, comp);
        AlnRec *p_al = wk->pin_get<AlnRec>("dl_alns", last);
        PS_HIP(hipMemcpyAsync(p_al, comp, (size_t)last * sizeof(AlnRec), hipMemcpyDeviceToHost, s));
        PS_HIP(hipStreamSynchronize(s));
        std::memcpy(alns.data(), p_al, (size_t)last * sizeof(AlnRec));
    }
}

__global__ void k_classify(const AlnRec *alns, int aln_cap, const int32_t *n_aln, const uint8_t *status, const int32_t *ids,
                           int n, int n_occ, uint8_t *cls_out)
{
    for (int r = blockIdx.x * blockDim.x + threadIdx.x; r < n; r += gridDim.x * blockDim.x) {
        uint8_t c = 0;
        if (status[r] != RS_OK) c = 3 | PS_CLS_HOST;
        else {
            const int na = n_aln[r];
            if (na > 0) {
                const AlnRec *al = alns + (size_t)r * aln_cap;
                const int best = al[0].score;
                int nb = 0; unsigned long long tot = 0;
                for (int j = 0; j < na; ++j) { if (al[j].score == best && nb == j) ++nb; tot += (unsigned long long)(al[j].l - al[j].k) + 1ull; }
                c = nb == 1 ? 1 : 2;
                if (c == 2 || (n_occ > 0 && tot >= 2 && tot <= (unsigned long long)n_occ + 1ull)) c |= PS_CLS_HOST;
            }
        }
        cls_out[ids[r]] = c;
    }
}
__global__ void k_gather_sub(const AlnRec *alns, int aln_cap, const int32_t *n_aln, const int32_t *local, int m, AlnRec *out, int32_t *n_out)
{
    for (int q = blockIdx.x * blockDim.x + threadIdx.x; q < m; q += gridDim.x * blockDim.x) {
        const int r = local[q]; int na = n_aln[r]; if (na > aln_cap) na = aln_cap;
        n_out[q] = na;
        for (int j = 0; j < na; ++j) out[(size_t)q * aln_cap + j] = alns[(size_t)r * aln_cap + j];
    }
}

__device__ __forceinline__ unsigned long long lcg_jump(unsigned long long x, unsigned long long t)
{
    const unsigned long long M = 0xFFFFFFFFFFFFULL;
    unsigned long long a = 0x5DEECE66DULL, c = 0xBULL, ra = 1, rc = 0;
    while (t) {
        if (t & 1) { ra = (ra * a) & M; rc = (rc * a + c) & M; }
        c = (c * a + c) & M; a = (a * a) & M;
        t >>= 1;
    }
    return (ra * x + rc) & M;
}

struct SelectArgs {
    const AlnRec *alns; int aln_cap; const int32_t *n_aln; const int32_t *ids; int n;
    const uint8_t *cls; const uint32_t *e_before; const uint32_t *h_before; const unsigned long long *hard_cum;
    unsigned long long draws_in;
    SelRec *sel; bwtint *rows; int *err;
};
struct MainPick { bwtint sa; int32_t c1, c2; int type, n_mm, n_gapo, n_gape, ref_shift, score; };
__host__ __device__ inline unsigned long long lcg48_next(unsigned long long x) { return (x * 0x5DEECE66DULL + 0xBULL) & 0xFFFFFFFFFFFFULL; }
__host__ __device__ inline int rule_choose_main(const AlnRec *al, int na, unsigned long long &x, MainPick &h)
{
    int cnt = 0, draws = 0, i;
    const int best = al[0].score;
    h.sa = 0; h.n_mm = h.n_gapo = h.n_gape = h.ref_shift = h.score = 0;
    for (i = 0; i < na; ++i) {
        const AlnRec p = al[i];
        if (p.score > best) break;
        const unsigned long long wdt = (unsigned long long)(p.l - p.k) + 1ull;
        x = lcg48_next(x); ++draws;
        if ((double)x * (1.0 / 281474976710656.0) * (double)(wdt + (unsigned long long)(long long)cnt) > (double)cnt) {
            h.n_mm = p.n_mm; h.n_gapo = p.n_gapo; h.n_gape = p.n_gape;
            h.ref_shift = (int)p.n_del - (int)p.n_ins; h.score = p.score;
            x = lcg48_next(x); ++draws;
            h.sa = p.k + (bwtint)((double)wdt * ((double)x * (1.0 / 281474976710656.0)));
        }
        cnt += (int)wdt;
    }
    h.c1 = cnt;
    for (; i < na; ++i) cnt += (int)((unsigned long long)(al[i].l - al[i].k) + 1ull);
    h.c2 = cnt - h.c1;
    h.type = h.c1 > 1 ? 2 : 1;
    return draws;
}

__global__ void k_select(SelectArgs a)
{
    for (int r = blockIdx.x * blockDim.x + threadIdx.x; r < a.n; r += gridDim.x * blockDim.x) {
        const int g = a.ids[r];
        const uint8_t c = a.cls[g];
        SelRec s; s.sa = 0; s.c1 = s.c2 = 0; s.type = 0; s.n_mm = s.n_gapo = s.n_gape = 0; s.ref_shift = 0; s.score = 0; s.pad[0] = s.pad[1] = 0;
        if (c == 1) {
            const AlnRec *al = a.alns + (size_t)r * a.aln_cap;
            const int na = a.n_aln[r];
            const unsigned int hb = a.h_before[g];
            const unsigned long long off = a.draws_in + 2ull * a.e_before[g] + (hb ? a.hard_cum[hb - 1] : 0ull);
            unsigned long long x = lcg_jump((11ull << 16) | 0x330Eull, off);
            if (lcg48_next(x) == 0) *a.err = 1;
            MainPick pk;
            (void)rule_choose_main(al, na, x, pk);
            s.sa = pk.sa; s.c1 = pk.c1; s.c2 = pk.c2; s.type = (uint8_t)pk.type;
            s.n_mm = (uint8_t)pk.n_mm; s.n_gapo = (uint8_t)pk.n_gapo; s.n_gape = (uint8_t)pk.n_gape; s.ref_shift = (int8_t)pk.ref_shift; s.score = (uint8_t)pk.score;
        }
        a.sel[g] = s;
        a.rows[g] = s.type ? s.sa : 0;
    }
}

struct PostArgs {
    const int32_t *ids; int n, len; const int32_t *lens; long long l_pac;
    const uint8_t *cls; const SelRec *sel; const bwtint *pos; FinRec *fin;
    int budget, profile, unit; const uint8_t *logn;
    const uint8_t *budget_by_len;
    RefineItem *items; int32_t *item_g; unsigned int *n_items;
};
__host__ __device__ inline long long rule_to_forward(long long pos_t, long long l_pac, int ref_len, int &strand)
{
    long long pos_f = pos_t;
    strand = 0;
    if (pos_f < l_pac && l_pac < pos_f + ref_len) return -1;
    const bool is_rev = pos_f >= l_pac;
    if (is_rev) pos_f = 2 * l_pac - 1 - pos_f;
    strand = !is_rev;
    if (is_rev) pos_f = pos_f + 1 < ref_len ? 0 : pos_f - ref_len + 1;
    return pos_f;
}
__host__ __device__ inline int rule_mapq(int c1, int c2, int n_mm, int score, int budget, bool profile, int unit, const uint8_t *logn)
{
    if (c1 == 0) return 23;
    if (c1 > 1) return 0;
    if (!profile) { if (n_mm == budget) return 25; }
    else if (budget * unit - score < unit) return 25;
    if (c2 == 0) return 37;
    const int lg = logn[c2 >= 255 ? 255 : c2];
    return 23 < lg ? 0 : 23 - lg;
}
static void mapq_logn_table(uint8_t logn[256])
{
    logn[0] = 0;
    for (int n = 1; n < 256; ++n) logn[n] = (uint8_t)(int)(4.343 * std::log((double)n) + 0.5);
}

__global__ void k_post(PostArgs a)
{
    for (int r = blockIdx.x * blockDim.x + threadIdx.x; r < a.n; r += gridDim.x * blockDim.x) {
        const int g = a.ids[r];
        FinRec f; f.pos = -1; f.strand = 0; f.mapq = 0; f.type = 0; f.pad[0] = f.pad[1] = f.pad[2] = f.pad[3] = f.pad[4] = 0;
        const SelRec s = a.sel[g];
        if (a.cls[g] == 1 && s.type != 0) {
            const int ref_len = (a.lens ? a.lens[r] : a.len) + s.ref_shift;
            int strand = 0;
            const long long p = rule_to_forward((long long)a.pos[g], a.l_pac, ref_len, strand);
            const int budget = (a.lens && a.budget_by_len) ? (int)a.budget_by_len[a.lens[r]] : a.budget;
            const int mq = rule_mapq(s.c1, s.c2, s.n_mm, (int)s.score, budget, a.profile != 0, a.unit, a.logn);
            f.pos = p; f.strand = (uint8_t)strand; f.mapq = (uint8_t)mq; f.type = p < 0 ? 0 : s.type;
            if (f.type != 0 && s.n_gapo) {
                const unsigned int q = atomicAdd(a.n_items, 1u);
                a.items[q] = RefineItem{r, (bwtint)p, (int32_t)s.ref_shift, strand};
                a.item_g[q] = g;
            }
        }
        a.fin[g] = f;
    }
}

void reserve_search_workspace(Ctx *ctx, int work_index)
{
    require_device(ctx->device);
    Work *wk = ctx->work_at(work_index);
    int dev_cus = 256;
    { hipDeviceProp_t p; if (hipGetDeviceProperties(&p, ctx->device) == hipSuccess && p.multiProcessorCount > 0) dev_cus = p.multiProcessorCount; }
    const uint32_t pool_cap = ctx->pool_cap[0];
    if (pool_cap > 65535) return;
    int blocks = ctx->bt_blocks > 0 ? ctx->bt_blocks : dev_cus * 4;
    const size_t per_lane = (size_t)pool_cap * 16, max_lanes = ((size_t)64 << 30) / per_lane;
    if ((size_t)blocks * 256 > max_lanes) blocks = (int)std::max<size_t>(1, max_lanes / 256);
    (void)wk->ws_get<uint8_t>("pool", (size_t)blocks * 256 * per_lane);
    if (pool_cap < 65535 && ctx->n_big > 0) {
        (void)wk->ws_get<uint8_t>("big_pool", (size_t)ctx->n_big * 65535 * 16);
        (void)wk->ws_get<uint32_t>("big_busy", (size_t)ctx->n_big);
    }
}

void batch_search(Batch &b)
{
    Ctx *ctx = b.ctx; Work *wk = b.wk; hipStream_t s = wk->stream;
    require_device(ctx->device);
    b.tm = Timing();
    auto t0 = Clock::now();
    const int64_t N = b.rs.n;
    b.d_stats.zero(s);
    for (int t = 0; t < 3; ++t) b.n_overflow[t] = 0;
    if (b.d_class.n < (size_t)N) b.d_class.alloc((size_t)N);
    for (Bin &bin : b.bins) {
        const int n = (int)bin.ids.size();
        bin.host_alns_valid = false;
        const int cap1 = (bin.len <= 40 && ctx->aln_cap_short > ctx->aln_cap[0]) ? ctx->aln_cap_short : ctx->aln_cap[0];
        if (bin.d_alns.n < (size_t)n * cap1 || bin.aln_cap != cap1) { bin.d_alns.alloc((size_t)n * cap1); bin.d_n_aln.alloc(n); bin.d_status.alloc(n); }
        bin.aln_cap = cap1;
        run_search(b, bin.md, n, bin.bases.p, bin.nmask.p, bin.ragged ? bin.d_lens.p : nullptr, ctx->pool_cap[0], bin.aln_cap, bin.d_alns.p, bin.d_n_aln.p, bin.d_status.p, true);
        uint8_t *h_status = wk->pin_get<uint8_t>("status", n);
        PS_HIP(hipMemcpyAsync(h_status, bin.d_status.p, (size_t)n, hipMemcpyDeviceToHost, s));
        hipLaunchKernelGGL(k_classify, dim3(std::min((n + 255) / 256, 4096)), dim3(256), 0, s, bin.d_alns.p, bin.aln_cap, bin.d_n_aln.p, bin.d_status.p,
                           bin.d_ids.p, n, ctx->opt.n_occ, b.d_class.p);
        PS_HIP(hipStreamSynchronize(s));
        bin.overflow.clear();
        std::vector<int32_t> todo;
        for (int r = 0; r < n; ++r) {
            if (h_status[r] == RS_OK) continue;
            if (h_status[r] == RS_BAD_SCORE) throw Error("internal: score outside the bucket range");
            todo.push_back(r);
        }
        std::vector<int32_t> deep;
        { std::vector<int32_t> keep; for (int32_t r : todo) (h_status[r] == RS_OVERFLOW_DEEP ? deep : keep).push_back(r); todo.swap(keep); }
        for (int tier = 1; tier < 3; ++tier) {
            if (tier == 2) { todo.insert(todo.end(), deep.begin(), deep.end()); std::sort(todo.begin(), todo.end()); deep.clear(); }
            if (todo.empty()) continue;
            b.n_overflow[tier] += (int64_t)todo.size();
            const int m = (int)todo.size();
            std::vector<uint32_t> hb((size_t)bin.n_bw * m), hm((size_t)bin.n_mw * m);
            for (int q = 0; q < m; ++q) {
                for (int wv = 0; wv < bin.n_bw; ++wv) hb[(size_t)wv * m + q] = bin.h_bases[(size_t)wv * n + todo[q]];
                for (int wv = 0; wv < bin.n_mw; ++wv) hm[(size_t)wv * m + q] = bin.h_nmask[(size_t)wv * n + todo[q]];
            }
            DevBuf<uint32_t> db, dm; db.alloc(hb.size()); dm.alloc(hm.size());
            db.upload(hb.data(), hb.size(), s); dm.upload(hm.data(), hm.size(), s);
            std::vector<int32_t> hl(m); DevBuf<int32_t> dl;
            if (bin.ragged) { for (int q = 0; q < m; ++q) hl[q] = bin.lens[todo[q]]; dl.alloc(m); dl.upload(hl.data(), m, s); }
            DevBuf<AlnRec> ta; DevBuf<int32_t> tn; DevBuf<uint8_t> ts;
            ta.alloc((size_t)m * ctx->aln_cap[tier]); tn.alloc(m); ts.alloc(m);
            run_search(b, bin.md, m, db.p, dm.p, bin.ragged ? dl.p : nullptr, ctx->pool_cap[tier], ctx->aln_cap[tier], ta.p, tn.p, ts.p);
            std::vector<uint8_t> st(m); ts.download(st.data(), m, s);
            std::vector<int32_t> na; std::vector<uint32_t> off; std::vector<AlnRec> al;
            download_alns(wk, m, ctx->aln_cap[tier], ta.p, tn.p, na, off, al);
            std::vector<int32_t> still;
            for (int q = 0; q < m; ++q) {
                if (st[q] == RS_BAD_SCORE) throw Error("internal: score outside the bucket range");
                if (st[q] != RS_OK) { still.push_back(todo[q]); continue; }
                bin.overflow[todo[q]] = std::vector<AlnRec>(al.begin() + off[q], al.begin() + off[q + 1]);
            }
            todo.swap(still);
        }
        if (!todo.empty()) throw Error("a read exceeded the largest search tier (stack or hit capacity)");
    }
    KStats hs[3];
    b.d_stats.download(hs, 3, s);
    auto tcl = Clock::now();
    b.h_class = (uint8_t *)b.p_class.get((size_t)N + 64);
    PS_HIP(hipMemcpyAsync(b.h_class, b.d_class.p, (size_t)N, hipMemcpyDeviceToHost, s));
    PS_HIP(hipStreamSynchronize(s));
    b.st_width = hs[0]; b.st_backtrack = hs[1];
    bool patched = false;
    for (Bin &bin : b.bins)
        for (auto &kv : bin.overflow) {
            const std::vector<AlnRec> &al = kv.second;
            int nb = 0;
            for (; nb < (int)al.size() && al[nb].score == al[0].score; ++nb) {}
            b.h_class[bin.ids[kv.first]] = (uint8_t)((al.empty() ? 0 : (nb == 1 ? 1 : 2)) | PS_CLS_HOST);
            patched = true;
        }
    if (patched) PS_HIP(hipMemcpyAsync(b.d_class.p, b.h_class, (size_t)N, hipMemcpyHostToDevice, s));
    b.sub.clear(); b.n_class1 = 0; b.n_hard = 0;
    {
        const int nt = par_threads((size_t)N, ctx->host_threads);
        std::vector<int64_t> ce(nt + 1, 0), ch(nt + 1, 0), cs(nt + 1, 0);
        par_for((size_t)N, ctx->host_threads, [&](size_t g0, size_t g1, int t) {
            int64_t e = 0, h = 0, sn = 0;
            for (size_t g = g0; g < g1; ++g) { const uint8_t c = b.h_class[g]; e += (c & 3) == 1; h += (c & 3) == 2; sn += (c & PS_CLS_HOST) != 0; }
            ce[t + 1] = e; ch[t + 1] = h; cs[t + 1] = sn;
        });
        for (int t = 0; t < nt; ++t) { ce[t + 1] += ce[t]; ch[t + 1] += ch[t]; cs[t + 1] += cs[t]; }
        b.n_class1 = ce[nt]; b.n_hard = ch[nt];
        b.sub.resize((size_t)cs[nt]);
        b.h_grp = (uint32_t *)b.p_grp.get((((size_t)N + 63) / 64 * 2 + 2) * sizeof(uint32_t));
        par_for((size_t)N, ctx->host_threads, [&](size_t g0, size_t g1, int t) {
            int64_t e = ce[t], h = ch[t]; size_t q = (size_t)cs[t];
            for (size_t g = g0; g < g1; ++g) {
                const uint8_t c = b.h_class[g];
                if ((g & 63) == 0) { b.h_grp[2 * (g >> 6)] = (uint32_t)e; b.h_grp[2 * (g >> 6) + 1] = (uint32_t)h; }
                if (c & PS_CLS_HOST) { SubRead &sr = b.sub[q++]; sr = SubRead(); sr.g = (int64_t)g; sr.cls = c & 3; sr.easy_before = e; sr.hard_before = h; }
                e += (c & 3) == 1; h += (c & 3) == 2;
            }
        });
        std::vector<std::vector<int32_t>> want(b.bins.size());
        std::vector<int32_t> slot(b.sub.size(), -1);
        for (size_t q = 0; q < b.sub.size(); ++q) {
            const SubRead &sr = b.sub[q];
            const int bi = b.read_bin[sr.g]; const Bin &bin = b.bins[bi];
            if (bin.overflow.empty() || !bin.overflow.count(b.read_local[sr.g])) { slot[q] = (int32_t)want[bi].size(); want[bi].push_back(b.read_local[sr.g]); }
        }
        b.sub_alns.resize(b.bins.size());
        std::vector<const AlnRec *> got(b.bins.size(), nullptr); std::vector<const int32_t *> got_n(b.bins.size(), nullptr);
        for (size_t bi = 0; bi < b.bins.size(); ++bi) {
            const int m = (int)want[bi].size();
            if (!m) continue;
            Bin &bin = b.bins[bi];
            int32_t *d_loc = wk->ws_get<int32_t>("sub_local", m); AlnRec *d_out = wk->ws_get<AlnRec>("sub_alns", (size_t)m * bin.aln_cap);
            int32_t *d_no = wk->ws_get<int32_t>("sub_n", m);
            PS_HIP(hipMemcpyAsync(d_loc, want[bi].data(), (size_t)m * 4, hipMemcpyHostToDevice, s));
            hipLaunchKernelGGL(k_gather_sub, dim3((m + 255) / 256), dim3(256), 0, s, bin.d_alns.p, bin.aln_cap, bin.d_n_aln.p, d_loc, m, d_out, d_no);
            if (!b.sub_alns[bi]) b.sub_alns[bi].reset(new PinBuf());
            const size_t bytes_al = (size_t)m * bin.aln_cap * sizeof(AlnRec);
            uint8_t *hp = (uint8_t *)b.sub_alns[bi]->get(bytes_al + (size_t)m * 4 + 64);
            PS_HIP(hipMemcpyAsync(hp, d_out, bytes_al, hipMemcpyDeviceToHost, s));
            PS_HIP(hipMemcpyAsync(hp + bytes_al, d_no, (size_t)m * 4, hipMemcpyDeviceToHost, s));
            got[bi] = reinterpret_cast<const AlnRec *>(hp); got_n[bi] = reinterpret_cast<const int32_t *>(hp + bytes_al);
        }
        PS_HIP(hipStreamSynchronize(s));
        par_for(b.sub.size(), ctx->host_threads, [&](size_t q0, size_t q1, int) {
            for (size_t q = q0; q < q1; ++q) {
                SubRead &sr = b.sub[q];
                const int bi = b.read_bin[sr.g]; Bin &bin = b.bins[bi];
                if (slot[q] < 0) { const std::vector<AlnRec> &v = bin.overflow.find(b.read_local[sr.g])->second; sr.alns = v.data(); sr.n_alns = (int32_t)v.size(); }
                else { sr.alns = got[bi] + (size_t)slot[q] * bin.aln_cap; sr.n_alns = got_n[bi][slot[q]]; }
            }
        });
    }
    b.tm.ms_classify = ms_since(tcl);
    b.searched = true; b.selected_hard = b.selected = b.located = false;
    b.tm.ms_total = ms_since(t0);
}

void Batch::ensure_host_alns()
{
    require_device(ctx->device);
    for (Bin &bin : bins) {
        if (bin.host_alns_valid) continue;
        download_alns(wk, (int)bin.ids.size(), bin.aln_cap, bin.d_alns.p, bin.d_n_aln.p, bin.h_n_aln, bin.h_off, bin.h_alns);
        for (auto &kv : bin.overflow) bin.h_n_aln[kv.first] = (int32_t)kv.second.size();
        bin.host_alns_valid = true;
    }
}
const AlnRec *Batch::alns_of(int64_t g, int &n)
{
    ensure_host_alns();
    const Bin &bin = bins[read_bin[g]];
    int32_t r = read_local[g];
    n = bin.h_n_aln[r];
    if (!bin.overflow.empty()) {
        auto it = bin.overflow.find(r);
        if (it != bin.overflow.end()) return it->second.data();
    }
    return bin.h_alns.data() + bin.h_off[r];
}

static int choose_main(const AlnRec *al, int na, Rng48 &rng, Hit &h)
{
    MainPick pk;
    unsigned long long x = rng.x;
    const int draws = rule_choose_main(al, na, x, pk);
    rng.x = x;
    h.sa = pk.sa; h.c1 = pk.c1; h.c2 = pk.c2; h.type = pk.type;
    h.n_mm = pk.n_mm; h.n_gapo = pk.n_gapo; h.n_gape = pk.n_gape; h.ref_shift = pk.ref_shift; h.score = pk.score;
    return draws;
}

void batch_select_hard(Batch &b, uint64_t draws_before, uint64_t *draws_after)
{
    if (!b.searched) throw Error("select before search");
    auto t0 = Clock::now();
    b.draws_in = draws_before;
    b.hard_draws_cum.assign((size_t)b.n_hard, 0);
    Rng48 rng(11);
    rng.jump(draws_before);
    uint64_t H = 0; int64_t e_prev = 0;
    for (SubRead &sr : b.sub) {
        if (sr.cls != 2) continue;
        rng.jump(2ull * (uint64_t)(sr.easy_before - e_prev));
        e_prev = sr.easy_before;
        sr.hit = Hit();
        H += (uint64_t)choose_main(sr.alns, sr.n_alns, rng, sr.hit);
        b.hard_draws_cum[(size_t)sr.hard_before] = H;
    }
    b.draws_out = draws_before + 2ull * (uint64_t)b.n_class1 + H;
    if (draws_after) *draws_after = b.draws_out;
    b.selected_hard = true;
    b.tm.ms_select += ms_since(t0); b.tm.ms_sel_hard = ms_since(t0);
}

void batch_select_easy(Batch &b, int threads)
{
    if (!b.selected_hard) throw Error("select_easy before select_hard");
    Ctx *ctx = b.ctx; Work *wk = b.wk; hipStream_t s = wk->stream;
    require_device(ctx->device);
    auto t0 = Clock::now();
    const int64_t N = b.rs.n;
    (void)threads;
    if (b.d_sel.n < (size_t)N) { b.d_sel.alloc((size_t)N); b.d_fin.alloc((size_t)N); b.d_rows.alloc((size_t)N + 1); b.d_pos.alloc((size_t)N + 1); b.d_eb.alloc((size_t)N); b.d_hb.alloc((size_t)N); }
    const double ms_alloc = ms_since(t0);
    {
        const size_t n_grp = ((size_t)N + 63) / 64;
        uint32_t *d_grp = wk->ws_get<uint32_t>("class_grp", 2 * n_grp + 2);
        PS_HIP(hipMemcpyAsync(d_grp, b.h_grp, 2 * n_grp * sizeof(uint32_t), hipMemcpyHostToDevice, s));
        launch_class_ranks(b.d_class.p, (long long)N, d_grp, b.d_eb.p, b.d_hb.p, s);
    }
    unsigned long long *d_cum = wk->ws_get<unsigned long long>("hard_cum", (size_t)b.n_hard + 1);
    if (b.n_hard) PS_HIP(hipMemcpyAsync(d_cum, b.hard_draws_cum.data(), (size_t)b.n_hard * 8, hipMemcpyHostToDevice, s));
    int *d_err = wk->ws_get<int>("sel_err", 4);
    PS_HIP(hipMemsetAsync(d_err, 0, 16, s));
    for (Bin &bin : b.bins) {
        SelectArgs a;
        a.alns = bin.d_alns.p; a.aln_cap = bin.aln_cap; a.n_aln = bin.d_n_aln.p; a.ids = bin.d_ids.p; a.n = (int)bin.ids.size();
        a.cls = b.d_class.p; a.e_before = b.d_eb.p; a.h_before = b.d_hb.p; a.hard_cum = d_cum; a.draws_in = b.draws_in;
        a.sel = b.d_sel.p; a.rows = b.d_rows.p; a.err = d_err;
// ... 251 lines not shown
```

para-suite_amd/csrc/ps_stage.hip:

```cpp
#include <hip/hip_runtime.h>
#include <stdexcept>
#include "ps_kernels.h"
#include "ps_budget.h"

namespace ps {

struct BinCounters { uint32_t c[4]; };

__device__ __forceinline__ uint32_t bins_fetch_add(BinCounters &b, int lane, int k, uint32_t n)
{
    const int owner = k & 63, j = k >> 6;
    uint32_t before;
    if (j == 0) { before = (uint32_t)__builtin_amdgcn_readlane((int)b.c[0], owner); if (lane == owner) b.c[0] += n; }
    else if (j == 1) { before = (uint32_t)__builtin_amdgcn_readlane((int)b.c[1], owner); if (lane == owner) b.c[1] += n; }
    else if (j == 2) { before = (uint32_t)__builtin_amdgcn_readlane((int)b.c[2], owner); if (lane == owner) b.c[2] += n; }
    else { before = (uint32_t)__builtin_amdgcn_readlane((int)b.c[3], owner); if (lane == owner) b.c[3] += n; }
    return before;
}
__device__ __forceinline__ uint32_t bins_take_tile(BinCounters &b, int lane, bool valid, int key)
{
    const unsigned long long lane_lt = (1ull << lane) - 1ull;
    unsigned long long todo = __ballot(valid);
    uint32_t place = 0;
    while (todo) {
        const int src = __builtin_amdgcn_readfirstlane(__ffsll(todo) - 1);
        const int k = __builtin_amdgcn_readlane(key, src);
        const bool mine = valid && key == k;
        const unsigned long long m = __ballot(mine);
        const uint32_t before = bins_fetch_add(b, lane, k, (uint32_t)__popcll(m));
        if (mine) place = before + (uint32_t)__popcll(m & lane_lt);
        todo &= ~m;
    }
    return place;
}
__device__ __forceinline__ uint32_t wave_inclusive_sum(uint32_t v, int lane)
{
#pragma unroll
    for (int o = 1; o < 64; o <<= 1) { const uint32_t u = (uint32_t)__shfl_up((int)v, o, 64); if (lane >= o) v += u; }
    return v;
}

__global__ void __launch_bounds__(64) k_sort_hist(const uint8_t *key, int n, int chunk, int n_wg, uint32_t *table)
{
    const int lane = threadIdx.x, wg = blockIdx.x;
    const long long beg = (long long)wg * chunk, end = beg + chunk < n ? beg + chunk : n;
    BinCounters b = {{0, 0, 0, 0}};
    for (long long at = beg; at < end; at += 64) {
        const long long i = at + lane;
        const bool valid = i < end;
        (void)bins_take_tile(b, lane, valid, valid ? (int)key[i] : 0);
    }
#pragma unroll
    for (int j = 0; j < 4; ++j) table[(size_t)(64 * j + lane) * n_wg + wg] = b.c[j];
}
__global__ void __launch_bounds__(64) k_sort_scan(uint32_t *table, int n_wg, uint32_t *totals)
{
    const int lane = threadIdx.x;
    uint32_t *row = table + (size_t)blockIdx.x * n_wg;
    const int per = (n_wg + 63) / 64, lo = lane * per, hi = lo + per < n_wg ? lo + per : n_wg;
    uint32_t sum = 0;
    for (int t = lo; t < hi; ++t) sum += row[t];
    const uint32_t incl = wave_inclusive_sum(sum, lane);
    uint32_t run = incl - sum;
    for (int t = lo; t < hi; ++t) { const uint32_t v = row[t]; row[t] = run; run += v; }
    if (lane == 63) totals[blockIdx.x] = incl;
}
__global__ void __launch_bounds__(64) k_sort_scatter(const uint8_t *key, int n, int chunk, int n_wg, const uint32_t *table, const uint32_t *totals, int32_t *order)
{
    const int lane = threadIdx.x, wg = blockIdx.x;
    const long long beg = (long long)wg * chunk, end = beg + chunk < n ? beg + chunk : n;
    BinCounters b;
    uint32_t below = 0;
#pragma unroll
    for (int j = 0; j < 4; ++j) {
        const uint32_t t = totals[64 * j + lane], incl = wave_inclusive_sum(t, lane);
        b.c[j] = below + (incl - t) + table[(size_t)(64 * j + lane) * n_wg + wg];
        below += (uint32_t)__builtin_amdgcn_readlane((int)incl, 63);
    }
    for (long long at = beg; at < end; at += 64) {
        const long long i = at + lane;
        const bool valid = i < end;
        const uint32_t place = bins_take_tile(b, lane, valid, valid ? (int)key[i] : 0);
        if (valid && place < (uint32_t)n) order[place] = (int32_t)i;
    }
}

size_t order_sort_tmp_words(int n) { (void)n; return (size_t)256 * PS_SORT_MAX_WG + 256; }
void launch_order_sort(const uint8_t *key, int n, uint32_t *tmp, int32_t *order, hipStream_t s)
{
    if (n <= 0) return;
    long long wgs = ((long long)n + 4095) / 4096;
    if (wgs > PS_SORT_MAX_WG) wgs = PS_SORT_MAX_WG;
    long long per = ((long long)n + wgs - 1) / wgs;
    per = (per + 63) / 64 * 64;
    const int chunk = (int)per, n_wg = (int)(((long long)n + per - 1) / per);
    uint32_t *table = tmp, *totals = tmp + (size_t)256 * PS_SORT_MAX_WG;
    hipLaunchKernelGGL(k_sort_hist, dim3(n_wg), dim3(64), 0, s, key, n, chunk, n_wg, table);
    hipLaunchKernelGGL(k_sort_scan, dim3(256), dim3(64), 0, s, table, n_wg, totals);
    hipLaunchKernelGGL(k_sort_scatter, dim3(n_wg), dim3(64), 0, s, key, n, chunk, n_wg, table, totals, order);
}

__global__ void __launch_bounds__(256) k_class_ranks(const uint8_t *cls, long long n, const uint32_t *grp, uint32_t *e_before, uint32_t *h_before)
{
    const int lane = threadIdx.x & 63;
    const unsigned long long lane_lt = (1ull << lane) - 1ull;
    const long long n_groups = (n + 63) >> 6, n_waves = ((long long)gridDim.x * blockDim.x) >> 6;
    for (long long q = ((long long)blockIdx.x * blockDim.x + threadIdx.x) >> 6; q < n_groups; q += n_waves) {
        const long long g = (q << 6) + lane;
        const int c = g < n ? (int)(cls[g] & 3) : 0;
        const unsigned long long m1 = __ballot(c == 1), m2 = __ballot(c == 2);
        if (g < n) {
            e_before[g] = grp[2 * q] + (uint32_t)__popcll(m1 & lane_lt);
            h_before[g] = grp[2 * q + 1] + (uint32_t)__popcll(m2 & lane_lt);
        }
    }
}
void launch_class_ranks(const uint8_t *cls, long long n, const uint32_t *grp, uint32_t *e_before, uint32_t *h_before, hipStream_t s)
{
    if (n <= 0) return;
    long long blocks = (n + 255) / 256;
    if (blocks > 2048) blocks = 2048;
    hipLaunchKernelGGL(k_class_ranks, dim3((unsigned int)blocks), dim3(256), 0, s, cls, n, grp, e_before, h_before);
}

}
```

para-suite_amd/csrc/ps_types.h:

```cpp
#pragma once
#include <stdint.h>
#include <stddef.h>

#ifdef __HIPCC__
#define PS_HD __host__ __device__ __forceinline__
#define PS_COLD __host__ __device__ inline __attribute__((noinline))
#else
#define PS_HD inline
#define PS_COLD inline
#endif

namespace ps {

typedef uint64_t bwtint;
static const bwtint PS_MAX_ROWS = (1ull << 33) - 64;

static const int PS_BLK_SYMS = 192;
struct OccBlock { uint32_t cnt[4]; uint32_t sym[12]; };

struct IndexView {
    const OccBlock *blocks;
    const uint32_t *sa;
    const uint32_t *sa_hi;
    const uint8_t  *pac;
    bwtint seq_len;
    bwtint primary;
    bwtint l_pac;
    bwtint L2[5];
    uint32_t n_blocks, n_sa;
    int sa_intv;
    const uint32_t *jump;
    int jump_levels;
};

struct Model {
    uint8_t u_mm[5][4], s_mm[5][4];
    uint32_t u_mm_pk[5], s_mm_pk[5];
    int32_t u_gapo_ins, s_gapo_ins, u_gapo_del, s_gapo_del, u_gape, s_gape;
    int32_t s_stop, u_tight, c_min, inv_c_min , max_units, n_buckets;
    int32_t max_gapo, max_gape, mode_gape, indel_end_skip, max_del_occ, max_entries;
    int32_t seed_len, max_seed_diff, max_top2, use_seed, len, profile;
};
static const int PS_MAX_BUCKETS = 128;
static const int PS_MAX_LEN = 250;

struct Entry {
    bwtint k, l;
    uint16_t score, units;
    uint8_t i, last_diff_pos, n_mm, n_gapo, n_gape, n_ins, n_del, state;
    uint32_t next;
};
static const uint32_t PS_NIL = 0xFFFFFFFFu;
enum { ST_M = 0, ST_I = 1, ST_D = 2 };

struct AlnRec {
    bwtint k, l;
    uint16_t score, units;
    uint8_t n_mm, n_gapo, n_gape, n_ins, n_del, pad[7];
};

enum { RS_OK = 0, RS_OVERFLOW_POOL = 1, RS_OVERFLOW_ALN = 2, RS_BAD_SCORE = 3,
       RS_OVERFLOW_DEEP = 4 };

struct KStats {
    unsigned long long occ_pairs, occ_same_blk, nodes, pushes, pops, lf_steps, iters, exact_steps;
};

static const int PS_RI_WORDS = 20;
struct BtArgs {
    IndexView ix;
    Model md;
    int n_reads, len, n_lanes;
    const int32_t *lens;
    const uint8_t *units_by_len;
    const uint32_t *bases; const uint32_t *nmask; int n_bw, n_mw;
    uint32_t *w; const uint32_t *cwb; const uint32_t *cswb;
    AlnRec *alns; int aln_cap; int32_t *n_aln; uint8_t *status;
    void *pool; uint32_t pool_cap;
    uint32_t *heads;
    int wide;
    uint8_t *big_pool; uint32_t big_cap, n_big; uint32_t *big_busy; uint32_t *big_next;
    uint32_t *queue;
    const int32_t *order;
    const uint8_t *est; const uint16_t *est_ab;
    int cap_est;
    uint32_t *read_iters;
    int hit_min;
    int fetch_min;
    KStats *stats;
};

}
```

Measured before the change: 8.718 million.

## Pre-pack per-read handout records and batch global loads in backtrack fetch/hit

Adds a handout kernel that packs each ordered read's id, length, unit budget and estimate into one 64-bit word. The backtrack fetch then does one load instead of chasing order, lens, units_by_len and est separately. The fetch and hit paths are rewritten to issue groups of global loads together before using them, with explicit address-space casts and a scalar-loaded argument copy. The alignment record is written as two 128-bit stores. Idle and drop counters are also added for stats, and the extra kernel and buffer add a little launch and memory overhead.

```diff
diff --git a/para-suite_amd/csrc/ps_capi.hip b/para-suite_amd/csrc/ps_capi.hip
--- a/para-suite_amd/csrc/ps_capi.hip
+++ b/para-suite_amd/csrc/ps_capi.hip
@@ -377,7 +377,7 @@
 int ps_batch_kstats(ps_batch *b, int which, ps_kstats *o)
 {
     PS_TRY
-        const KStats &k = which == 0 ? b->b->st_width : (which == 1 ? b->b->st_backtrack : b->b->st_sa2pos);
+        const KStats &k = which == 0 ? b->b->st_width : (which == 1 ? b->b->st_backtrack : (which == 3 ? b->b->st_idle : b->b->st_sa2pos));
         o->occ_pairs = k.occ_pairs; o->occ_same_blk = k.occ_same_blk; o->nodes = k.nodes; o->pushes = k.pushes; o->pops = k.pops;
         o->lf_steps = k.lf_steps; o->iters = k.iters; o->exact_steps = k.exact_steps; return 0;
     PS_CATCH_INT
diff --git a/para-suite_amd/csrc/ps_core.h b/para-suite_amd/csrc/ps_core.h
--- a/para-suite_amd/csrc/ps_core.h
+++ b/para-suite_amd/csrc/ps_core.h
@@ -117,7 +117,8 @@
 }
 PS_HD uint32_t width32(bwtint k, bwtint l) { const bwtint w = l - k + 1; return w > 0xFFFFFFFFull ? 0xFFFFFFFFu : (uint32_t)w; }
 
-struct LaneStats { uint32_t pairs, same, nodes, pushes, pops, iters, exact, lf; };
+struct LaneStats { uint32_t pairs, same, nodes, pushes, pops, iters, exact, lf;
+                   uint32_t wait_fetch, wait_hit, dropped; };
 
 PS_HD void occ_pair4(const OccBlock *blocks, bwtint primary, bwtint k, bwtint l, uint32_t ck[4], uint32_t cl[4], LaneStats &st)
 {
diff --git a/para-suite_amd/csrc/ps_kernels.h b/para-suite_amd/csrc/ps_kernels.h
--- a/para-suite_amd/csrc/ps_kernels.h
+++ b/para-suite_amd/csrc/ps_kernels.h
@@ -69,6 +69,7 @@
 void launch_refine(const RefineArgs &a, int n_blocks, hipStream_t s);
 size_t order_sort_tmp_words(int n);
 void launch_order_sort(const uint8_t *key, int n, uint32_t *tmp, int32_t *order, hipStream_t s);
+void launch_handout(const int32_t *order, int n, const int32_t *lens, int len, const uint8_t *units_by_len, int max_units, const uint8_t *est, unsigned long long *handout, hipStream_t s);
 void launch_class_ranks(const uint8_t *cls, long long n, const uint32_t *grp, uint32_t *e_before, uint32_t *h_before, hipStream_t s);
 
 }
diff --git a/para-suite_amd/csrc/ps_kernels.hip b/para-suite_amd/csrc/ps_kernels.hip
--- a/para-suite_amd/csrc/ps_kernels.hip
+++ b/para-suite_amd/csrc/ps_kernels.hip
@@ -271,6 +271,11 @@
         st.pops = lane == 0 ? (uint32_t)(clk.tm[2] >> 6) : 0; st.exact = lane == 0 ? (uint32_t)(clk.tm[3] >> 6) : 0;
 #endif
         flush_stats(a.stats, st);
+        if (a.idle) {
+            const unsigned long long v[3] = {st.wait_fetch, st.wait_hit, st.dropped};
+#pragma unroll
+            for (int j = 0; j < 3; ++j) { const unsigned long long s = wave_sum(v[j]); if (lane == 0 && s) atomicAdd(a.idle + j, s); }
+        }
     } else {
         st.nodes = st.pushes = st.pops = st.iters = st.exact = st.lf = 0;
         flush_stats(a.stats, st);
diff --git a/para-suite_amd/csrc/ps_narrow.h b/para-suite_amd/csrc/ps_narrow.h
--- a/para-suite_amd/csrc/ps_narrow.h
+++ b/para-suite_amd/csrc/ps_narrow.h
@@ -48,7 +48,7 @@
     L.kr = L.lr = L.wa = L.wb = 0; L.ctl = (uint32_t)M_FETCH; L.r = 0; L.lim = 0; L.nsb = 0;
     L.n_phantom = 0; L.fh = 0xffffu; L.bm0 = L.bm1 = 0; L.rn0 = L.rn1 = 0;
 }
-PS_HD void ls_init(LaneStats &st) { st.pairs = st.same = st.nodes = st.pushes = st.pops = st.iters = st.exact = st.lf = 0; }
+PS_HD void ls_init(LaneStats &st) { st.pairs = st.same = st.nodes = st.pushes = st.pops = st.iters = st.exact = st.lf = 0; st.wait_fetch = st.wait_hit = st.dropped = 0; }
 PS_HD uint32_t ps_mul24(uint32_t x, uint32_t y)
 {
 #ifdef __HIP_DEVICE_COMPILE__
@@ -171,107 +171,245 @@
     L.ctl = nl_set_mode(L.ctl, M_FETCH);
 }
 
-PS_COLD void nt_hit(const BtArgs &a, NLane &L, BtMem &m)
-{
-    const Model &md = a.md;
+#ifdef __HIP_DEVICE_COMPILE__
+#define PS_AS_LDS(T, p) ((__attribute__((address_space(3))) T *)(p))
+#else
+#define PS_AS_LDS(T, p) ((T *)(p))
+#define PS_AS_GLOBAL(T, p) ((const T *)(p))
+#define PS_AS_GLOBAL_W(T, p) ((T *)(p))
+#endif
+struct NtCold {
+    const unsigned long long *handout; const int32_t *order, *lens; const uint8_t *units_by_len, *est;
+    const uint32_t *bases, *nmask, *cwb, *cswb, *jump;
+    uint32_t *w; AlnRec *alns; int32_t *n_aln; uint8_t *status;
+    bwtint seq_len, L2[4];
+    uint32_t n_reads, u_n;
+    int len, aln_cap, cap_est, jump_levels, seed_len, max_units, u_tight, n_buckets, profile, mode_gape, max_top2;
+};
+PS_HD void nt_cold_load(NtCold &k, const BtArgs &a_)
+{
+#ifdef __HIP_DEVICE_COMPILE__
+    const unsigned long long at = reinterpret_cast<unsigned long long>(&a_);
+    const uint32_t lo = (uint32_t)__builtin_amdgcn_readfirstlane((int)(uint32_t)at), hi = (uint32_t)__builtin_amdgcn_readfirstlane((int)(uint32_t)(at >> 32));
+    const __attribute__((address_space(4))) BtArgs &a = *(const __attribute__((address_space(4))) BtArgs *)((unsigned long long)lo | ((unsigned long long)hi << 32));
+#else
+    const BtArgs &a = a_;
+#endif
+    k.handout = a.handout; k.order = a.order; k.lens = a.lens; k.units_by_len = a.units_by_len; k.est = a.est;
+    k.bases = a.bases; k.nmask = a.nmask; k.cwb = a.cwb; k.cswb = a.cswb; k.jump = a.ix.jump;
+    k.w = a.w; k.alns = a.alns; k.n_aln = a.n_aln; k.status = a.status;
+    k.seq_len = a.ix.seq_len;
+    for (int c = 0; c < 4; ++c) k.L2[c] = a.ix.L2[c];
+    k.n_reads = (uint32_t)a.n_reads; k.u_n = a.md.u_mm_pk[4] & 0xffu;
+    k.len = a.len; k.aln_cap = a.aln_cap; k.cap_est = a.cap_est; k.jump_levels = a.ix.jump_levels; k.seed_len = a.md.seed_len;
+    k.max_units = a.md.max_units; k.u_tight = a.md.u_tight; k.n_buckets = a.md.n_buckets; k.profile = a.md.profile;
+    k.mode_gape = a.md.mode_gape; k.max_top2 = a.md.max_top2;
+}
+PS_HD void nt_cold_finish_read(const NtCold &k, NLane &L)
+{
+    *PS_AS_GLOBAL_W(int32_t, k.n_aln + L.r) = nl_n_aln(L.ctl);
+    *PS_AS_GLOBAL_W(uint8_t, k.status + L.r) = (uint8_t)nl_status(L.ctl);
+    L.ctl = nl_set_mode(L.ctl, M_FETCH);
+}
+#ifdef __HIP_DEVICE_COMPILE__
+#define PS_LANDED4(a, b, c, d) asm volatile("" : "+v"(a), "+v"(b), "+v"(c), "+v"(d))
+#else
+#define PS_LANDED4(a, b, c, d) do { } while (0)
+#endif
+
+static const int NT_SHADOW_GROUP = 4;
+PS_HD void nt_hit_body(const BtArgs &a, NLane &L, BtMem &m)
+{
+    NtCold k; nt_cold_load(k, a);
     const uint32_t c = nw_c(L.wb);
-    if (a.ix.jump && c != NW_ROOT_C) {
+    const size_t n_reads = k.n_reads, r = (size_t)(uint32_t)L.r;
+    if (k.jump && c != NW_ROOT_C) {
         const int d = nt_depth(nl_len(L), L.wa, L.wb);
-        if (d < a.ix.jump_levels) {
-            const uint32_t *ps = a.ix.jump + (size_t)(jump_level_off(d - 1) + (L.kr >> 2)) * PS_JUMP_SLOT_WORDS;
-            L.kr = ps[2 * c] + 1u; L.lr = ps[2 * c + 1];
-        }
-    }
-    const bwtint base = c == NW_ROOT_C ? (a.ix.seq_len & ~(bwtint)0xFFFFFFFFull) : a.ix.L2[c];
-    const bwtint k = base + L.kr, l = base + L.lr;
+        if (d < k.jump_levels) {
+            const uint32_t *ps = k.jump + (size_t)(jump_level_off(d - 1) + (L.kr >> 2)) * PS_JUMP_SLOT_WORDS + 2 * c;
+            const uint32_t pk = *PS_AS_GLOBAL(uint32_t, ps), pl = *PS_AS_GLOBAL(uint32_t, ps + 1);
+            L.kr = pk + 1u; L.lr = pl;
+        }
+    }
+    const bwtint base = c == NW_ROOT_C ? (k.seq_len & ~(bwtint)0xFFFFFFFFull) : (c == 0 ? k.L2[0] : c == 1 ? k.L2[1] : c == 2 ? k.L2[2] : k.L2[3]);
+    const bwtint kk = base + L.kr, l = base + L.lr;
     const int score = nw_score(L.wb), n_gapo = nw_gapo(L.wa);
-    const int units = md.profile ? score : nw_mm(L.wa) + n_gapo + (md.mode_gape ? nw_gape(L.wa) : 0);
+    const int units = k.profile ? score : nw_mm(L.wa) + n_gapo + (k.mode_gape ? nw_gape(L.wa) : 0);
     const int n_aln = nl_n_aln(L.ctl);
     if (n_aln == 0) {
         if (units > nl_est(L)) { nt_restart_without_estimate(a, L, m); return; }
-        int t = units + md.u_tight;
+        int t = units + k.u_tight;
         const int own = nl_max_units(L);
         t = t > own ? own : t;
         L.lim = (L.lim & 0x00FF0000u) | (uint32_t)score | ((uint32_t)t << 8);
     }
     if (score == nl_best_score(L)) {
-        const unsigned long long s = (unsigned long long)(L.lim >> 24) + (unsigned long long)(l - k) + 1ull;
+        const unsigned long long s = (unsigned long long)(L.lim >> 24) + (unsigned long long)(l - kk) + 1ull;
         L.lim = (L.lim & 0x00FFFFFFu) | ((s > 255ull ? 255u : (uint32_t)s) << 24);
-    } else if ((int)(L.lim >> 24) > md.max_top2) { nt_finish_read(a, L); return; }
-    AlnRec *out = a.alns + (size_t)L.r * a.aln_cap;
+    } else if ((int)(L.lim >> 24) > k.max_top2) { nt_cold_finish_read(k, L); return; }
+    AlnRec *out = k.alns + r * (size_t)k.aln_cap;
     if (n_gapo) {
-        for (int j = 0; j < n_aln; ++j)
-            if (out[j].k == k && out[j].l == l) return;
-    }
-    {
-        const uint32_t shadow = a.ix.seq_len > 0xFFFFFFFFull ? 0xFFFFFFFFu : (uint32_t)a.ix.seq_len;
-        uint32_t x = (uint32_t)(l - k + 1), j = 0, prev = 0;
+        bool dup = false;
+        for (int j0 = 0; j0 < n_aln && !dup; j0 += 4) {
+            bwtint ok[4], ol[4];
+#pragma unroll
+            for (int u = 0; u < 4; ++u) {
+                const int j = j0 + u < n_aln ? j0 + u : n_aln - 1;
+                ok[u] = *PS_AS_GLOBAL(bwtint, &out[j].k); ol[u] = *PS_AS_GLOBAL(bwtint, &out[j].l);
+            }
+#pragma unroll
+            for (int u = 0; u < 4; ++u) dup = dup || (ok[u] == kk && ol[u] == l);
+        }
+        if (dup) return;
+    }
+    {
+        const uint32_t shadow = k.seq_len > 0xFFFFFFFFull ? 0xFFFFFFFFu : (uint32_t)k.seq_len;
+        uint32_t x = (uint32_t)(l - kk + 1), j = 0, prev = 0;
         const int lim = nw_ldp(L.wa);
-        for (int i = 0; i < lim; ++i) {
-            size_t off = (size_t)i * a.n_reads + L.r;
-            uint32_t w = a.w[off];
-            int bid = m.cw[i] & 0x7f;
-            if (w > x) { w -= x; a.w[off] = w; }
-            else if (w == x) {
-                if (bid > 1 && nl_phantom(L)) L.ctl = nl_set_status(L.ctl, RS_OVERFLOW_POOL);
-                bid = 1; w = shadow - (++j); a.w[off] = w;
+        uint32_t *const wr = k.w + r;
+        for (int i0 = 0; i0 < lim; i0 += NT_SHADOW_GROUP) {
+            uint32_t wv[NT_SHADOW_GROUP]; uint8_t cb[NT_SHADOW_GROUP];
+#pragma unroll
+            for (int u = 0; u < NT_SHADOW_GROUP; ++u) {
+                const int i = i0 + u < lim ? i0 + u : lim - 1;
+                wv[u] = *PS_AS_GLOBAL(uint32_t, wr + (size_t)i * n_reads);
+                cb[u] = *PS_AS_LDS(uint8_t, m.cw + i);
             }
-            m.cw[i] = cw_pack(bid, i > 0 && w == prev);
-            prev = w;
+#pragma unroll
+            for (int u = 0; u < NT_SHADOW_GROUP; u += 4) PS_LANDED4(wv[u], wv[u + 1], wv[u + 2], wv[u + 3]);
+#pragma unroll
+            for (int u = 0; u < NT_SHADOW_GROUP; ++u) {
+                const int i = i0 + u;
+                if (i < lim) {
+                    uint32_t w = wv[u];
+                    int bid = cb[u] & 0x7f;
+                    if (w > x) { w -= x; *PS_AS_GLOBAL_W(uint32_t, wr + (size_t)i * n_reads) = w; }
+                    else if (w == x) {
+                        if (bid > 1 && nl_phantom(L)) L.ctl = nl_set_status(L.ctl, RS_OVERFLOW_POOL);
+                        bid = 1; w = shadow - (++j); *PS_AS_GLOBAL_W(uint32_t, wr + (size_t)i * n_reads) = w;
+                    }
+                    *PS_AS_LDS(uint8_t, m.cw + i) = cw_pack(bid, i > 0 && w == prev);
+                    prev = w;
+                }
+            }
         }
         if (lim > 0) {
-            uint32_t w = a.w[(size_t)lim * a.n_reads + L.r];
-            m.cw[lim] = cw_pack(m.cw[lim] & 0x7f, w == prev);
-        }
-    }
-    if (n_aln >= a.aln_cap) { L.ctl = nl_set_status(L.ctl, RS_OVERFLOW_ALN); nt_finish_read(a, L); return; }
+            const uint32_t w = *PS_AS_GLOBAL(uint32_t, wr + (size_t)lim * n_reads);
+            *PS_AS_LDS(uint8_t, m.cw + lim) = cw_pack(*PS_AS_LDS(uint8_t, m.cw + lim) & 0x7f, w == prev);
+        }
+    }
+    if (n_aln >= k.aln_cap) { L.ctl = nl_set_status(L.ctl, RS_OVERFLOW_ALN); nt_cold_finish_read(k, L); return; }
+#ifdef __HIP_DEVICE_COMPILE__
+    static_assert(sizeof(AlnRec) == 32 && offsetof(AlnRec, l) == 8 && offsetof(AlnRec, score) == 16 && offsetof(AlnRec, units) == 18 && offsetof(AlnRec, n_mm) == 20 &&
+                  offsetof(AlnRec, n_ins) == 23 && offsetof(AlnRec, n_del) == 24, "the packed record below is AlnRec's layout");
+    {
+        ps_u32x4 v0, v1;
+        v0.x = (uint32_t)kk; v0.y = (uint32_t)(kk >> 32); v0.z = (uint32_t)l; v0.w = (uint32_t)(l >> 32);
+        v1.x = (uint32_t)(uint16_t)score | ((uint32_t)(uint16_t)units << 16);
+        v1.y = (uint32_t)nw_mm(L.wa) | ((uint32_t)n_gapo << 8) | ((uint32_t)nw_gape(L.wa) << 16) | ((uint32_t)nw_ins(L.wb) << 24);
+        v1.z = (uint32_t)nw_del(L.wb); v1.w = 0;
+        *PS_AS_GLOBAL_W(ps_u32x4, out + n_aln) = v0;
+        *(PS_AS_GLOBAL_W(ps_u32x4, out + n_aln) + 1) = v1;
+    }
+#else
     AlnRec rec;
-    rec.k = k; rec.l = l; rec.score = (uint16_t)score; rec.units = (uint16_t)units;
+    rec.k = kk; rec.l = l; rec.score = (uint16_t)score; rec.units = (uint16_t)units;
     rec.n_mm = (uint8_t)nw_mm(L.wa); rec.n_gapo = (uint8_t)n_gapo; rec.n_gape = (uint8_t)nw_gape(L.wa);
     rec.n_ins = (uint8_t)nw_ins(L.wb); rec.n_del = (uint8_t)nw_del(L.wb);
-    for (int j = 0; j < 7; ++j) rec.pad[j] = 0;
+    for (int j2 = 0; j2 < 7; ++j2) rec.pad[j2] = 0;
     out[n_aln] = rec;
+#endif
     L.ctl += 1u << 16;
 }
 
-PS_COLD bool nt_fetch(const BtArgs &a, NLane &L, BtMem &m, int q)
-{
-    const Model &md = a.md;
-    const int r = a.order ? a.order[q] : q;
-    const int len = a.lens ? a.lens[r] : a.len;
-    L.r = r;
+PS_COLD void nt_hit(const BtArgs &a, NLane &L_, BtMem &m_)
+{
+    NLane L = L_; BtMem m = m_;
+    nt_hit_body(a, L, m);
+    L_ = L;
+}
+
+PS_HD unsigned long long handout_pack(uint32_t r, int len, int units, int est)
+{
+    return (unsigned long long)r | ((unsigned long long)(len & 0xff) << 32) | ((unsigned long long)(units & 0xff) << 40) | ((unsigned long long)(est & 0xff) << 48);
+}
+static const int NT_FETCH_WORDS = 28;
+
+PS_HD bool nt_fetch_body(const BtArgs &a, NLane &L, BtMem &m, int q)
+{
+    NtCold k; nt_cold_load(k, a);
+    uint32_t r = (uint32_t)q;
+    int len = k.len, max_units = k.max_units, est = 0;
+    const bool rec = k.handout != nullptr;
+    if (rec) {
+        const unsigned long long hr = *PS_AS_GLOBAL(unsigned long long, k.handout + q);
+        r = (uint32_t)hr; len = (int)((hr >> 32) & 0xffu); max_units = (int)((hr >> 40) & 0xffu); est = (int)((hr >> 48) & 0xffu);
+    } else if (k.order) r = (uint32_t)*PS_AS_GLOBAL(int32_t, k.order + q);
+    const size_t n_reads = k.n_reads;
+    const int w_cw = lm_ncw(k.len), w_csw = lm_ncsw(k.seed_len), w_rb = (k.len + 15) >> 4, w_nm = (k.len + 31) >> 5;
+    const bool nm_regs = lm_nmask_in_regs(k.len);
+    const int total = w_cw + w_csw + w_rb + (nm_regs ? 0 : w_nm);
+    uint32_t nm0 = 0, nm1 = 0, len_w = 0, est_w = 0;
+    int nNw = 0;
+    for (int base = 0; base < total; base += NT_FETCH_WORDS) {
+        uint32_t d[NT_FETCH_WORDS];
+#pragma unroll
+        for (int u = 0; u < NT_FETCH_WORDS; ++u) {
+            int x = base + u < total ? base + u : total - 1;
+            const uint32_t *src = k.cwb;
+            if (x >= w_cw) { x -= w_cw; src = k.cswb; if (x >= w_csw) { x -= w_csw; src = k.bases; if (x >= w_rb) { x -= w_rb; src = k.nmask; } } }
+            d[u] = *PS_AS_GLOBAL(uint32_t, src + (size_t)x * n_reads + r);
+        }
+        if (base == 0) {
+            if (nm_regs) { nm0 = *PS_AS_GLOBAL(uint32_t, k.nmask + r); nm1 = *PS_AS_GLOBAL(uint32_t, k.nmask + (w_nm > 1 ? n_reads : (size_t)0) + r); }
+            if (!rec && k.lens) len_w = (uint32_t)*PS_AS_GLOBAL(int32_t, k.lens + r);
+            if (!rec && k.est) est_w = *PS_AS_GLOBAL(uint8_t, k.est + r);
+        }
+#pragma unroll
+        for (int u = 0; u < NT_FETCH_WORDS; u += 4) PS_LANDED4(d[u], d[u + 1], d[u + 2], d[u + 3]);
+        if (base == 0) {
+            PS_LANDED4(nm0, nm1, len_w, est_w);
+            if (!rec && k.lens) len = (int)len_w;
+            if (!rec) est = (int)est_w;
+        }
+#pragma unroll
+        for (int u = 0; u < NT_FETCH_WORDS; ++u) {
+            const int x = base + u;
+            if (x < total) {
+                *PS_AS_LDS(uint32_t, reinterpret_cast<uint32_t *>(m.cw) + x) = d[u];
+                const int pm = x - (w_cw + w_csw + w_rb);
+                if (pm >= 0 && pm < ((len + 31) >> 5)) nNw += (int)ps_popc(d[u]);
+            }
+        }
+    }
+    if (!rec && k.lens && k.units_by_len) max_units = (int)*PS_AS_GLOBAL(uint8_t, k.units_by_len + len);
+    L.r = (int)r;
     L.ctl = (uint32_t)M_FETCH;
     L.n_phantom = 0xFF000000u;
-    const int max_units = (a.lens && a.units_by_len) ? (int)a.units_by_len[len] : md.max_units;
     L.lim = 0xffu | ((uint32_t)max_units << 8) | ((uint32_t)len << 16);
-    {
-        const int ncw = lm_ncw(len), ncsw = lm_ncsw(md.seed_len);
-        uint32_t *cw32 = reinterpret_cast<uint32_t *>(m.cw), *csw32 = reinterpret_cast<uint32_t *>(m.csw);
-        for (int p = 0; p < ncw; ++p) cw32[p] = a.cwb[(size_t)p * a.n_reads + r];
-        for (int p = 0; p < ncsw; ++p) csw32[p] = a.cswb[(size_t)p * a.n_reads + r];
-        const int nbw = (len + 15) >> 4;
-        for (int p = 0; p < nbw; ++p) m.rb[p] = a.bases[(size_t)p * a.n_reads + r];
-    }
-    int nNu = 0;
-    L.rn0 = L.rn1 = 0;
     const int nmw = (len + 31) >> 5;
-    for (int p = 0; p < nmw; ++p) {
-        uint32_t w = a.nmask[(size_t)p * a.n_reads + r];
-        if (lm_nmask_in_regs(a.len)) { if (p == 0) L.rn0 = w; else L.rn1 = w; }
-        else m.rn[p] = w;
-        nNu += (int)ps_popc(w) * (int)(md.u_mm_pk[4] & 0xffu);
-    }
-    if (nNu > max_units) { nt_finish_read(a, L); return false; }
-    L.kr = 0; L.lr = (uint32_t)a.ix.seq_len; L.wa = (uint32_t)len; L.wb = NW_ROOT_C << 6;
+    L.rn0 = nm_regs && nmw > 0 ? nm0 : 0u; L.rn1 = nm_regs && nmw > 1 ? nm1 : 0u;
+    if (nm_regs) nNw = (int)ps_popc(L.rn0) + (int)ps_popc(L.rn1);
+    if (nNw * (int)k.u_n > max_units) { nt_cold_finish_read(k, L); return false; }
+    L.kr = 0; L.lr = (uint32_t)k.seq_len; L.wa = (uint32_t)len; L.wb = NW_ROOT_C << 6;
     L.ctl |= NL_HAVE_CUR;
     L.nsb = 0; L.bm0 = L.bm1 = 0; L.fh = 0xffffu;
     {
         int e = 255;
-        if (a.cap_est) { e = (int)a.est[r] - (a.cap_est - 1); if (e < 0) e = 0; }
-        L.n_phantom = (uint32_t)(e + md.u_tight < max_units ? e : 255) << 24;
-    }
-    nt_heads_init(m, md.n_buckets);
+        if (k.cap_est) { e = est - (k.cap_est - 1); if (e < 0) e = 0; }
+        L.n_phantom = (uint32_t)(e + k.u_tight < max_units ? e : 255) << 24;
+    }
+    {
+        uint32_t *hw = reinterpret_cast<uint32_t *>(m.heads16);
+        for (int p = 0; p < (k.n_buckets + 1) >> 1; ++p) *PS_AS_LDS(uint32_t, hw + p) = 0xFFFFFFFFu;
+    }
     return true;
+}
+
+PS_COLD bool nt_fetch(const BtArgs &a, NLane &L, BtMem &m_, int q)
+{
+    BtMem m = m_;
+    return nt_fetch_body(a, L, m, q);
 }
 
 PS_HD uint32_t nt_slot(NLane &L)
@@ -320,13 +458,13 @@
     if (mode == M_EXIT || mode == M_GROW) return 0;
     if (STATS) ++st.iters;
     if (mode == M_HIT) {
-        if (!serve_hit) return 0;
+        if (!serve_hit) { if (STATS) ++st.wait_hit; return 0; }
         L.ctl = nl_set_mode(L.ctl, M_POP);
         { NLane t = L; nt_hit(a, t, m); L = t; }
         return 0;
     }
     if (mode == M_FETCH) {
-        if (fetch_r < 0) return 0;
+        if (fetch_r < 0) { if (STATS) ++st.wait_fetch; return 0; }
         if (fetch_r >= (int)h.n_reads) { L.ctl = nl_set_mode(L.ctl, M_EXIT); return 0; }
         { NLane t = L; const bool ok = nt_fetch(a, t, m, fetch_r); L = t; if (!ok) return 0; }
         L.ctl = nl_set_mode(L.ctl, M_POP);
@@ -345,9 +483,9 @@
         const int score = nw_score(L.wb), i1 = nw_i(L.wa);
         if (score > nl_best_score(L) + h.s_stop()) { nt_finish_read(a, L); return 0; }
         const int rem = nl_max_units(L) - nt_units(h, L.wa, L.wb);
-        if (rem < 0) return 0;
+        if (rem < 0) { if (STATS) ++st.dropped; return 0; }
         const int mleft = (int)(ps_mul24((uint32_t)rem, h.inv_c_min) >> 16);
-        if (i1 > 0 && mleft < (int)(m.cw[i1 - 1] & 0x7f)) return 0;
+        if (i1 > 0 && mleft < (int)(m.cw[i1 - 1] & 0x7f)) { if (STATS) ++st.dropped; return 0; }
         if (i1 == 0) { L.ctl = nl_set_mode(L.ctl, M_HIT); return 0; }
         const int st_ = nw_state(L.wa);
         mode = (mleft == 0 && (st_ == ST_M || h.mode_gape() || nw_gape(L.wa) == h.max_gape())) ? M_EXACT : M_EXPAND;
diff --git a/para-suite_amd/csrc/ps_pipeline.h b/para-suite_amd/csrc/ps_pipeline.h
--- a/para-suite_amd/csrc/ps_pipeline.h
+++ b/para-suite_amd/csrc/ps_pipeline.h
@@ -113,7 +113,7 @@
     int64_t n_class1 = 0, n_hard = 0;
     std::vector<uint64_t> hard_draws_cum;
     uint64_t draws_in = 0, draws_out = 0;
-    DevBuf<KStats> d_stats; KStats st_width{}, st_backtrack{}, st_sa2pos{};
+    DevBuf<KStats> d_stats; KStats st_width{}, st_backtrack{}, st_sa2pos{}, st_idle{};
     Timing tm;
     int64_t n_overflow[3] = {0, 0, 0};
     bool searched = false, selected_hard = false, selected = false, located = false;
diff --git a/para-suite_amd/csrc/ps_pipeline.hip b/para-suite_amd/csrc/ps_pipeline.hip
--- a/para-suite_amd/csrc/ps_pipeline.hip
+++ b/para-suite_amd/csrc/ps_pipeline.hip
@@ -222,7 +222,7 @@
         bin.bases.upload(bin.h_bases.data(), bin.h_bases.size(), wk->stream);
         bin.nmask.upload(bin.h_nmask.data(), bin.h_nmask.size(), wk->stream);
     }
-    b->d_stats.alloc(3);
+    b->d_stats.alloc(4);
     PS_HIP(hipStreamSynchronize(wk->stream));
 }
 std::unique_ptr<Batch> batch_create(Ctx *ctx, ReadSet &&rs_in)
@@ -278,6 +278,15 @@
     t_width.emplace(s); launch_width(wa, s); PS_HIP(hipGetLastError()); t_width->mark(); ++b.tm.n_width_launches;
     const bool wide = launch_is_wide(md, pool_cap);
     const int32_t *d_order = nullptr; const uint8_t *d_est = nullptr; const uint16_t *d_est_ab = nullptr;
+    const unsigned long long *d_handout = nullptr;
+    const uint8_t *d_units_by_len = nullptr;
+    if (d_lens) {
+        uint8_t *tab = wk->pin_get<uint8_t>("units_by_len_h", 256);
+        for (int l2 = 0; l2 < 256; ++l2) { const int u = budget_diffs(ctx->opt, l2) * (ctx->opt.profile ? ctx->opt.unit : 1); tab[l2] = (uint8_t)(u > 255 ? 255 : u); }
+        uint8_t *d_tab = wk->ws_get<uint8_t>("units_by_len", 256);
+        PS_HIP(hipMemcpyAsync(d_tab, tab, 256, hipMemcpyHostToDevice, s));
+        d_units_by_len = d_tab;
+    }
     if (!wide) {
         const char *eo = std::getenv("PS_ORDER");
         const int mode = eo ? std::atoi(eo) : 1;
@@ -324,9 +333,12 @@
                 launch_effort_model(em, s);
             }
             launch_order_sort(key, n, wk->ws_get<uint32_t>("order_tmp", order_sort_tmp_words(n)), order, s);
+            unsigned long long *handout = wk->ws_get<unsigned long long>("handout", (size_t)n);
+            launch_handout(order, n, d_lens, len, d_units_by_len, md.max_units, est, handout, s);
             PS_HIP(hipGetLastError());
             t_order->mark();
-            d_order = order; d_est = est;
+            d_order = order; d_est = est; d_handout = handout;
+            if (const char *e = std::getenv("PS_HANDOUT")) if (std::atoi(e) == 0) d_handout = nullptr;
         }
     }
     int dev_cus = 256;
@@ -348,19 +360,14 @@
     PS_HIP(hipMemsetAsync(queue, 0, 64, s));
     BtArgs a; std::memset(&a, 0, sizeof a);
     a.ix = ctx->ix.view; a.md = md; a.n_reads = n; a.len = len; a.lens = d_lens; a.n_lanes = n_lanes;
-    if (d_lens) {
-        uint8_t *tab = wk->pin_get<uint8_t>("units_by_len_h", 256);
-        for (int l2 = 0; l2 < 256; ++l2) { const int u = budget_diffs(ctx->opt, l2) * (ctx->opt.profile ? ctx->opt.unit : 1); tab[l2] = (uint8_t)(u > 255 ? 255 : u); }
-        uint8_t *d_tab = wk->ws_get<uint8_t>("units_by_len", 256);
-        PS_HIP(hipMemcpyAsync(d_tab, tab, 256, hipMemcpyHostToDevice, s));
-        a.units_by_len = d_tab;
-    }
+    a.units_by_len = d_units_by_len;
     a.bases = d_bases; a.nmask = d_nmask; a.n_bw = (len + 15) / 16; a.n_mw = (len + 31) / 32;
     a.w = w; a.cwb = cwb; a.cswb = cswb;
     a.alns = alns; a.aln_cap = aln_cap; a.n_aln = n_aln; a.status = status;
     a.pool = pool; a.pool_cap = pool_cap; a.heads = heads; a.wide = wide ? 1 : 0; a.stats = b.d_stats.p + 1;
+    a.idle = wide ? nullptr : reinterpret_cast<unsigned long long *>(b.d_stats.p + 3);
     a.queue = queue; a.fetch_min = ctx->fetch_min; a.hit_min = ctx->hit_min;
-    a.order = d_order; a.est = d_est; a.est_ab = d_est_ab;
+    a.order = d_order; a.est = d_est; a.est_ab = d_est_ab; a.handout = d_handout;
     a.cap_est = (first_tier && !wide && d_est && md.profile && !(std::getenv("PS_CAP") && std::atoi(std::getenv("PS_CAP")) == 0)) ? 1 : 0;
     if (a.cap_est) if (const char *e = std::getenv("PS_CAP_BIAS")) a.cap_est += std::max(0, std::min(200, std::atoi(e)));
     if (const char *e = std::getenv("PS_FETCH_MIN")) a.fetch_min = std::max(1, std::atoi(e));
@@ -646,13 +653,13 @@
         }
         if (!todo.empty()) throw Error("a read exceeded the largest search tier (stack or hit capacity)");
     }
-    KStats hs[3];
-    b.d_stats.download(hs, 3, s);
+    KStats hs[4];
+    b.d_stats.download(hs, 4, s);
     auto tcl = Clock::now();
     b.h_class = (uint8_t *)b.p_class.get((size_t)N + 64);
     PS_HIP(hipMemcpyAsync(b.h_class, b.d_class.p, (size_t)N, hipMemcpyDeviceToHost, s));
     PS_HIP(hipStreamSynchronize(s));
-    b.st_width = hs[0]; b.st_backtrack = hs[1];
+    b.st_width = hs[0]; b.st_backtrack = hs[1]; b.st_idle = hs[3];
     bool patched = false;
     for (Bin &bin : b.bins)
         for (auto &kv : bin.overflow) {
diff --git a/para-suite_amd/csrc/ps_stage.hip b/para-suite_amd/csrc/ps_stage.hip
--- a/para-suite_amd/csrc/ps_stage.hip
+++ b/para-suite_amd/csrc/ps_stage.hip
@@ -1,6 +1,7 @@
 #include <hip/hip_runtime.h>
 #include <stdexcept>
 #include "ps_kernels.h"
+#include "ps_narrow.h"
 #include "ps_budget.h"
 
 namespace ps {
@@ -100,6 +101,24 @@
     hipLaunchKernelGGL(k_sort_scatter, dim3(n_wg), dim3(64), 0, s, key, n, chunk, n_wg, table, totals, order);
 }
 
+__global__ void __launch_bounds__(256) k_handout(const int32_t *order, int n, const int32_t *lens, int len, const uint8_t *units_by_len, int max_units,
+                                                 const uint8_t *est, unsigned long long *handout)
+{
+    for (long long q = (long long)blockIdx.x * blockDim.x + threadIdx.x; q < n; q += (long long)gridDim.x * blockDim.x) {
+        const int r = order[q];
+        const int l = lens ? lens[r] : len;
+        const int u = (lens && units_by_len) ? (int)units_by_len[l & 0xff] : max_units;
+        handout[q] = handout_pack((uint32_t)r, l, u, est ? (int)est[r] : 0);
+    }
+}
+void launch_handout(const int32_t *order, int n, const int32_t *lens, int len, const uint8_t *units_by_len, int max_units, const uint8_t *est, unsigned long long *handout, hipStream_t s)
+{
+    if (n <= 0) return;
+    long long blocks = ((long long)n + 255) / 256;
+    if (blocks > 2048) blocks = 2048;
+    hipLaunchKernelGGL(k_handout, dim3((unsigned int)blocks), dim3(256), 0, s, order, n, lens, len, units_by_len, max_units, est, handout);
+}
+
 __global__ void __launch_bounds__(256) k_class_ranks(const uint8_t *cls, long long n, const uint32_t *grp, uint32_t *e_before, uint32_t *h_before)
 {
     const int lane = threadIdx.x & 63;
diff --git a/para-suite_amd/csrc/ps_types.h b/para-suite_amd/csrc/ps_types.h
--- a/para-suite_amd/csrc/ps_types.h
+++ b/para-suite_amd/csrc/ps_types.h
@@ -83,11 +83,13 @@
     uint32_t *queue;
     const int32_t *order;
     const uint8_t *est; const uint16_t *est_ab;
+    const unsigned long long *handout;
     int cap_est;
     uint32_t *read_iters;
     int hit_min;
     int fetch_min;
     KStats *stats;
+    unsigned long long *idle;
 };
 
 }
```

New measurement: 8.457 million. -3.0%, worse.
